# jzi040941/PercepNet

Measured on AMD Instinct MI355X. Metric: real-time 48 kHz streams (10 ms frames), whole job, higher is better.
Workload: dtype f32; 1 GPU; configs[2]: 65536 concurrent 48 kHz streams per MI355X, fp32 network as MFMA GEMM; streams_per_gpu=65536, frame_samples=480, nn_mode=mfma_f32, weights=torch.manual_seed(1234) default-init PercepNet in nnet_data.h layout, parallelism=streams sharded over 1 GPU(s), one process per GPU, no data-path collective, io=int16 PCM in, int16 PCM + g|r rows out, resident in HBM, distributed=none (plain process)

## Files before the change

percepnet_amd/build.py:

```python
import os
import subprocess
import sys

HERE = os.path.dirname(os.path.abspath(__file__))
CSRC = os.path.join(HERE, "csrc")
LIBDIR = os.path.join(HERE, "lib")
LIB = os.path.join(LIBDIR, "libpercepnet_hip.so")
RUN = os.path.join(LIBDIR, "percepnet_run")
EXPORT_MAP = os.path.join(CSRC, "libpercepnet_hip.map")
SOURCES = ["pn_tables.cpp", "pn_model.cpp", "pn_pack.cpp", "pn_dsp_fe.hip", "pn_dsp_fe_g2.hip", "pn_dsp_fe_split_s.hip", "pn_dsp_fe_split_p.hip", "pn_dsp.hip", "pn_outstage.hip", "pn_nn.hip", "pn_nn_small.hip", "pn_nn_x3.hip", "pn_nn_d.hip", "pn_nn_n48.hip", "pn_targets.hip", "pn_state.hip", "pn_active.hip", "pn_stream_state.hip", "pn_context.cpp", "pn_selftest.cpp", "pn_host_pipe.cpp", "pn_stream_state.cpp", "pn_network.cpp",
           "pn_featgen.cpp", "pn_rate.hip", "pn_rate_mix.hip", "pn_rate_plc.hip", "pn_rate_agc.hip", "pn_rate_lim.hip", "pn_rate.cpp", "rnnoise_compat.cpp"]
FLAGS = ["--offload-arch=gfx950", "-O3", "-std=c++17", "-ffp-contract=off", "-fPIC", "-fvisibility=hidden",
         "-Wall", "-Wno-unused-function", "-Wno-unused-variable", "-Wno-unused-value", "-Wno-unused-result"]


EXTRA_FLAGS = {"pn_nn_x3.hip": ["-fno-slp-vectorize", "-mllvm", "-pragma-unroll-threshold=1000000"],
               "pn_nn_d.hip": ["-fno-slp-vectorize"]}


def _hipcc():
    for c in (os.environ.get("HIPCC"), "/opt/rocm/bin/hipcc", "hipcc"):
        if c and (os.path.isabs(c) and os.path.exists(c) or not os.path.isabs(c)):
            return c
    raise RuntimeError("hipcc not found")


EXPECTED_HIP = "7.2"

RESOURCE_LIMITS = {"pn_fe_spec_in_kernel": (0, 0), "pn_fe_spec_out_kernel": (0, 40), "pn_fe_pitch_kernel": (0, 48),
                   "pn_backend_kernel": (0, 16),
                   "pn_gru_x3_kernel": (0, 0), "pn_dense_x3_kernel": (0, 0),
                   "pn_gru_d_kernel": (0, 0),
                   "pn_rate_": (0, 0)}
RESOURCE_SOURCES = ("pn_dsp_fe_split_s.hip", "pn_dsp_fe_split_p.hip", "pn_dsp.hip", "pn_nn_x3.hip", "pn_nn_d.hip", "pn_rate.hip", "pn_rate_mix.hip", "pn_rate_plc.hip", "pn_rate_agc.hip", "pn_rate_lim.hip")


def parse_resource_remarks(text):
    import re
    out, cur = {}, None
    for line in text.splitlines():
        m = re.search(r"remark: .*Function Name: (\S+)", line)
        if m:
            name = m.group(1)
            mm = re.match(r"_Z\d+(pn_[a-z0-9_]+)", name)
            cur = out.setdefault(name, {"kernel": mm.group(1) if mm else name})
            continue
        m = re.search(r"remark: .*?\s+(VGPRs|AGPRs|ScratchSize \[bytes/lane\]|Occupancy \[waves/SIMD\]|LDS Size \[bytes/block\]|VGPRs Spill|SGPRs Spill): (\d+)", line)
        if m and cur is not None:
            cur[m.group(1).split(" [")[0]] = int(m.group(2))
    return out


def check_resources(remarks):
    bad = []
    for name, r in remarks.items():
        for prefix, (max_agpr, max_scratch) in RESOURCE_LIMITS.items():
            if r["kernel"].startswith(prefix):
                if r.get("AGPRs", 0) > max_agpr or r.get("ScratchSize", 0) > max_scratch:
                    bad.append(f"{r['kernel']}: {r.get('VGPRs')} VGPRs, {r.get('AGPRs')} AGPRs, {r.get('ScratchSize')} B/lane scratch "
                               f"(limits: {max_agpr} AGPRs, {max_scratch} B) [{name}]")
    return bad


LLVM_BIN = "/opt/rocm/lib/llvm/bin"
GATED_OBJECTS = ("pn_dsp_fe_split_p",)


def disassemble_device_code(obj_path):
    import shutil
    import tempfile
    objdump = os.path.join(LLVM_BIN, "llvm-objdump")
    if not os.path.exists(objdump):
        objdump = shutil.which("llvm-objdump")
    if not objdump:
        raise RuntimeError("llvm-objdump not found: the disassembly gate cannot run")
    with tempfile.TemporaryDirectory() as d:
        local = os.path.join(d, os.path.basename(obj_path))
        shutil.copy(obj_path, local)
        subprocess.run([objdump, "--offloading", local], cwd=d, capture_output=True, text=True, check=True)
        cos = [f for f in os.listdir(d) if "amdgcn" in f]
        if not cos:
            raise RuntimeError(f"no device code object in {obj_path}")
        return subprocess.run([objdump, "-d", os.path.join(d, cos[0])], capture_output=True, text=True, check=True).stdout


def _vregs(op):
    import re
    m = re.fullmatch(r"v(\d+)", op)
    if m:
        return {int(m.group(1))}
    m = re.fullmatch(r"v\[(\d+):(\d+)\]", op)
    return set(range(int(m.group(1)), int(m.group(2)) + 1)) if m else set()


def check_dpp_and_waitcnt(disasm):
    import re
    bad = []
    func, ins = None, []
    funcs = {}
    for line in disasm.splitlines():
        m = re.match(r"^[0-9a-f]+ <([^>]+)>:", line)
        if m:
            func = m.group(1); ins = funcs.setdefault(func, [])
            continue
        t = line.split("//")[0].strip()
        if func is None or not t or t.startswith("."):
            continue
        parts = t.split(None, 1)
        ops = [o.strip() for o in re.split(r",\s*(?![^\[]*\])", parts[1])] if len(parts) > 1 else []
        ins.append((parts[0], ops, t))
    for func, ins in funcs.items():
        for i, (mn, ops, text) in enumerate(ins):
            if "_dpp" not in mn or len(ops) < 2:
                continue
            src0 = _vregs(ops[1].split()[0])
            if not src0:
                continue
            states, j = 0, i - 1
            while j >= 0 and states < 2:
                pm, pops, ptext = ins[j]
                if pm.startswith("v_") and pops and (_vregs(pops[0].split()[0]) & src0) and not pm.startswith(("v_cmp", "v_nop")):
                    bad.append(f"{func}: `{ptext}` writes the DPP-routed src0 of `{text}` only {states} wait state(s) earlier (need 2)")
                    break
                states += (int(pops[0], 0) + 1) if (pm == "s_nop" and pops) else 1
                j -= 1
        if "pn_fe_pitch_kernel" in func:
            pk = [i for i, x in enumerate(ins) if x[0] == "v_pk_mul_f32"]
            if pk:
                for mn, ops, text in ins[pk[0]:pk[-1] + 1]:
                    if mn.startswith(("s_load_", "s_buffer_load")):
                        bad.append(f"{func}: scalar load `{text}` inside the packed coarse loop (its hand-counted s_waitcnt lgkmcnt(4) assumes LDS reads only)")
    return bad


def toolchain_info(hipcc):
    try:
        out = subprocess.run([hipcc, "--version"], capture_output=True, text=True).stdout
    except OSError as e:
        return f"hipcc --version failed: {e}"
    ver = next((l.split(":", 1)[1].strip() for l in out.splitlines() if l.startswith("HIP version")), "?")
    if not ver.startswith(EXPECTED_HIP):
        print(f"[percepnet_amd.build] WARNING: hipcc reports HIP {ver}; the kernels were validated with HIP {EXPECTED_HIP}.x "
              f"(MFMA-drain and loop back-edge hazards, DESIGN.md): run the GPU parity tests before trusting this build",
              file=sys.stderr, flush=True)
    return out.strip()


def _obj(dirname, src):
    stem, ext = src.rsplit(".", 1)
    return os.path.join(dirname, stem + ("_host" if ext == "cpp" and stem + ".hip" in SOURCES else "") + ".o")


def _stale(target, deps):
    if not os.path.exists(target):
        return True
    t = os.path.getmtime(target)
    return any(os.path.getmtime(d) > t for d in deps)


def build_variant(name, defines, verbose=False, only=None):
    vdir = os.path.join(LIBDIR, "variants", name)
    os.makedirs(vdir, exist_ok=True)
    hipcc = _hipcc()
    objs = []
    for src in SOURCES:
        if only is not None and src not in only:
            objs.append(_obj(LIBDIR, src))
            continue
        o = _obj(vdir, src)
        cmd = [hipcc] + FLAGS + EXTRA_FLAGS.get(src, []) + list(defines) + (["-x", "hip"] if src.endswith(".cpp") else []) + \
              ["-c", os.path.join(CSRC, src), "-o", o]
        if verbose:
            print(" ".join(cmd), flush=True)
        subprocess.check_call(cmd)
        objs.append(o)
    lib = os.path.join(vdir, "libpercepnet_hip.so")
    subprocess.check_call([hipcc, "--offload-arch=gfx950", "-shared", "-fPIC", "-Wl,--version-script=" + EXPORT_MAP, "-o", lib] + objs)
    return lib


def build(force=False, verbose=True):
    os.makedirs(LIBDIR, exist_ok=True)
    hipcc = _hipcc()
    deps = [os.path.join(CSRC, f) for f in os.listdir(CSRC)] + [
        os.path.join(HERE, "..", "include", "percepnet_hip.h"),
        os.path.join(HERE, "..", "include", "percepnet_nnet_data.h")]
    objs = []
    resources = {}
    for src in SOURCES:
        s = os.path.join(CSRC, src)
        o = _obj(LIBDIR, src)
        rlog = o + ".resources.txt"
        if force or _stale(o, deps) or (src in RESOURCE_SOURCES and not os.path.exists(rlog)):
            cmd = [hipcc] + FLAGS + EXTRA_FLAGS.get(src, []) + (["-x", "hip"] if src.endswith(".cpp") else []) + ["-c", s, "-o", o]
            if src in RESOURCE_SOURCES:
                cmd.insert(-4, "-Rpass-analysis=kernel-resource-usage")
            if verbose:
                print(" ".join(cmd), flush=True)
            if src in RESOURCE_SOURCES:
                r = subprocess.run(cmd, capture_output=True, text=True)
                if r.returncode:
                    sys.stderr.write(r.stderr)
                    raise subprocess.CalledProcessError(r.returncode, cmd)
                open(rlog, "w").write("\n".join(l for l in r.stderr.splitlines() if "remark:" in l) + "\n")
            else:
                subprocess.check_call(cmd)
        if src in RESOURCE_SOURCES and os.path.exists(rlog):
            resources.update(parse_resource_remarks(open(rlog).read()))
        objs.append(o)
    bad = check_resources(resources)
    if bad:
        raise RuntimeError("register hygiene gate (build.RESOURCE_LIMITS) failed:\n  " + "\n  ".join(bad))
    for base in GATED_OBJECTS:
        o = os.path.join(LIBDIR, base + ".o")
        stamp = o + ".isa_gate_ok"
        if force or _stale(stamp, [o]):
            viol = check_dpp_and_waitcnt(disassemble_device_code(o))
            if viol:
                raise RuntimeError("disassembly gate (build.check_dpp_and_waitcnt) failed — rebuild with -DPN_FP_DPP_ASM=0 -DPN_FP_COARSE_PK=0 or "
                                   "fix the sequence:\n  " + "\n  ".join(viol[:20]))
            open(stamp, "w").write("ok\n")
    if force or _stale(LIB, objs + [EXPORT_MAP]):
        cmd = [hipcc, "--offload-arch=gfx950", "-shared", "-fPIC", "-Wl,--version-script=" + EXPORT_MAP, "-o", LIB] + objs
        if verbose:
            print(" ".join(cmd), flush=True)
        subprocess.check_call(cmd)
    for name in ("percepnet_run", "percepnet_featgen"):
        cli, exe = os.path.join(CSRC, name + ".cpp"), os.path.join(LIBDIR, name)
        if os.path.exists(cli) and (force or _stale(exe, [cli, LIB])):
            cmd = [hipcc, "--offload-arch=gfx950", "-O2", "-std=c++17", cli, "-o", exe, "-L" + LIBDIR,
                   "-lpercepnet_hip", "-Wl,-rpath,$ORIGIN", "-lpthread"]
            if verbose:
                print(" ".join(cmd), flush=True)
            subprocess.check_call(cmd)
    with open(os.path.join(LIBDIR, "BUILD_INFO.txt"), "w") as f:
        f.write(toolchain_info(hipcc) + "\nflags: " + " ".join(FLAGS) + "\n")
        f.write("DSP kernel resources (hipcc -Rpass-analysis=kernel-resource-usage):\n")
        for name, r in sorted(resources.items(), key=lambda kv: kv[1]["kernel"]):
            f.write(f"  {r['kernel']}: VGPRs {r.get('VGPRs')} AGPRs {r.get('AGPRs')} scratch {r.get('ScratchSize')} B/lane "
                    f"LDS {r.get('LDS Size')} B/block occupancy {r.get('Occupancy')} waves/SIMD  [{name[:60]}]\n")
    return LIB


if __name__ == "__main__":
    build(force="--force" in sys.argv)
    print(LIB)
```

percepnet_amd/csrc/pn_context.cpp:

```cpp
#include "pn_context.h"
#include <stdio.h>
#include <float.h>
#include <math.h>

extern "C" int pn_device_count(void) { int n = 0; return hipGetDeviceCount(&n) == hipSuccess ? n : 0; }


static thread_local bool g_last_alloc_oom = false;
bool &last_alloc_oom() { return g_last_alloc_oom; }
int dev_alloc_into(std::vector<void *> &allocs, size_t &total, hipStream_t stream, void **p, size_t bytes, bool zero) {
  static const bool guard = getenv("PERCEPNET_GUARD") != NULL;
  const size_t pad = guard ? (1u << 20) : 0, body = (bytes + 255) & ~(size_t)255;
  {
    const hipError_t e = hipMalloc(p, guard ? body + pad : bytes);
    if (e != hipSuccess) {
      g_last_alloc_oom = (e == hipErrorOutOfMemory);
      (void)hipGetLastError();
      pn_set_error("hipMalloc(%zu bytes) failed: %s", bytes, hipGetErrorString(e));
      return -1;
    }
  }
  allocs.push_back(*p);
  total += bytes;
  if (zero) PN_HIP_CHECK(hipMemsetAsync(*p, 0, bytes, stream));
  if (guard) PN_HIP_CHECK(hipMemsetAsync((char *)*p + body, 0xFF, pad, stream));
  return 0;
}
#define DEV_ALLOC(ptr, count, zero) \
  do { if (dev_alloc(c, (void **)&(ptr), sizeof(*(ptr)) * (size_t)(count), zero)) goto fail; } while (0)
int tables_upload(std::vector<void *> &allocs, size_t &total, hipStream_t stream, PnTables **tables, float **tansig) {
  PnTables *ht = new PnTables();
  hipError_t e = hipSuccess;
  int rc = pn_build_tables(ht);
  if (!rc) rc = dev_alloc_into(allocs, total, stream, (void **)tables, sizeof(PnTables), false);
  if (!rc) e = hipMemcpyAsync(*tables, ht, sizeof(PnTables), hipMemcpyHostToDevice, stream);
  if (!rc && e == hipSuccess && tansig) {
    rc = dev_alloc_into(allocs, total, stream, (void **)tansig, sizeof(ht->tansig), false);
    if (!rc) e = hipMemcpyAsync(*tansig, ht->tansig, sizeof(ht->tansig), hipMemcpyHostToDevice, stream);
  }
  const hipError_t es = hipStreamSynchronize(stream);
  if (e == hipSuccess) e = es;
  if (!rc && e != hipSuccess) { pn_set_error("table upload failed: %s", hipGetErrorString(e)); rc = -1; }
  delete ht;
  return rc;
}

static int zero_state(pn_ctx *c) {
  for (const pn_ctx::StateBuf &b : c->st) {
    PN_HIP_CHECK(hipMemsetAsync(b.p, 0, b.words * 4, c->stream));
    if (b.sh) PN_HIP_CHECK(hipMemsetAsync(b.sh, 0, b.words * 2 * shadow_halfs_per_element(c), c->stream));
  }
  if (c->lam_mu) PN_HIP_CHECK(hipMemsetAsync(c->lam_mu, 0, (size_t)c->B * sizeof(float2), c->stream));
  c->atten_db.assign(c->B, INFINITY); c->n_limited = 0;
  c->t = 0; c->tn = 0;
  return 0;
}
extern "C" void pn_ctx_destroy(pn_ctx *c) {
  if (!c) return;
  DeviceGuard _dg(c->device);
  hipStreamSynchronize(c->stream);
  pipe_destroy(c);
  for (int k = 1; k < 4; k++) if (c->chain_stream[k]) { hipStreamSynchronize(c->chain_stream[k]); hipStreamDestroy(c->chain_stream[k]); if (c->chain_join[k]) hipEventDestroy(c->chain_join[k]); }
  if (c->chain_fork) hipEventDestroy(c->chain_fork);
  for (auto &e : c->events) { hipEventDestroy(e.a); hipEventDestroy(e.b); }
  for (hipEvent_t e : c->event_pool) hipEventDestroy(e);
  for (void *p : c->allocs) hipFree(p);
  for (pn_ctx::IdRing *r : {&c->ids, &c->act.ids})
    for (auto &sl : r->slot) { if (sl.h) hipHostFree(sl.h); if (sl.ev) hipEventDestroy(sl.ev); }
  weights_release(c);
  if (c->own_stream) hipStreamDestroy(c->stream);
  delete c;
}

extern "C" pn_ctx *pn_ctx_create(const pn_model *model, int device, int n_streams, int nn_mode, void *hip_stream) {
  return ctx_create(model, device, n_streams, nn_mode, hip_stream, true, NULL);
}

int open_device(int device, void *hip_stream, DeviceGuard &guard, hipStream_t *stream, bool *own_stream) {
  int ndev = 0;
  if (hipGetDeviceCount(&ndev) != hipSuccess || ndev <= 0) {
    pn_set_error("no HIP device available (this library has no CPU fallback)");
    return -1;
  }
  if (device < 0 || device >= ndev) { pn_set_error("device %d out of range (%d devices)", device, ndev); return -1; }
  guard.enter(device);
  if (!guard.ok) { pn_set_error("hipSetDevice(%d) failed", device); return -1; }
  *stream = (hipStream_t)hip_stream; *own_stream = !hip_stream;
  if (!hip_stream && hipStreamCreateWithFlags(stream, hipStreamNonBlocking) != hipSuccess) { pn_set_error("hipStreamCreate failed"); return -1; }
  return 0;
}

pn_ctx *ctx_create(const pn_model *model, int device, int n_streams, int nn_mode, void *hip_stream, bool selftest, const PnPlan *plan) {
  if (!model) { pn_set_error("NULL model"); return NULL; }
  if (n_streams < 1) { pn_set_error("n_streams must be >= 1"); return NULL; }
  if (nn_mode != PN_NN_MFMA && nn_mode != PN_NN_STRICT && nn_mode != PN_NN_MFMA_F16 && nn_mode != PN_NN_MFMA_X3) { pn_set_error("bad nn_mode %d", nn_mode); return NULL; }
  DeviceGuard _dg; hipStream_t stream; bool own_stream;
  if (open_device(device, hip_stream, _dg, &stream, &own_stream)) return NULL;
  pn_ctx *c = new pn_ctx();
  c->stream = stream; c->own_stream = own_stream;
  c->device = device; c->B = n_streams; c->Bp = ((size_t)n_streams + 255) / 256 * 256; c->nn_mode = nn_mode; c->plan = plan ? *plan : pn_plan_for(n_streams, nn_mode);
  c->t = 0; c->tn = 0; c->bytes = 0; c->profiling = false;
  memset(c->fam_ms, 0, sizeof(c->fam_ms)); memset(c->fam_n, 0, sizeof(c->fam_n));
  memset(c->L, 0, sizeof(c->L));
  const size_t B = n_streams, Bp = c->Bp;
  float *base[PN_ST_COUNT];
  if (tables_upload(c->allocs, c->bytes, c->stream, &c->tables, &c->tansig)) goto fail;
  for (int e = 0; e < PN_ST_COUNT; e++) {
    pn_ctx::StateBuf &b = c->st[e];
    const PnStateSize z = pn_state_size(pn_kState[e], pn_kState[e].padded ? Bp : B);
    b.words = z.words; b.slot_stride = z.slot_stride;
    DEV_ALLOC(b.p, b.words, false);
    base[e] = b.p;
  }
  c->side = pn_dsp_side(base, nullptr, B);
  for (int e = 0; e < PN_ST_COUNT; e++)
    if (pn_state_shadowed(e, c->plan, nn_mode)) DEV_ALLOC(c->st[e].sh, shadow_halfs_per_element(c) * c->st[e].words, false);
  DEV_ALLOC(c->io_in, B * PN_FRAME, false);
  DEV_ALLOC(c->io_out, B * PN_FRAME, false);
  if (zero_state(c)) goto fail;
  for (int li = 0; li < PN_NLAYERS; li++) { c->geom[li] = model->L[li]; c->geom[li].bias = c->geom[li].w = c->geom[li].rw = NULL; }
  if (weights_acquire(c, model)) goto fail;
  if (hipStreamSynchronize(c->stream) != hipSuccess) { pn_set_error("initial upload failed"); goto fail; }
  if (selftest && (nn_mode == PN_NN_MFMA_X3 || nn_mode == PN_NN_MFMA_F16)) {
    const char *e = getenv("PERCEPNET_X3_SATCOUNT");
    c->x3_sat = e && atoi(e);
  }
  if (selftest && nn_mode != PN_NN_STRICT && nn_selftest(c)) goto fail;
  if (selftest && dsp_selftest(c)) goto fail;
  if (c->x3_sat && pn_x3_sat_set(1)) { pn_set_error("cannot enable the operand-saturation counter"); goto fail; }
  if (c->plan.chains > 1 && chain_streams_init(c)) goto fail;
  return c;
fail:
  pn_ctx_destroy(c);
  return NULL;
}

extern "C" int pn_ctx_reset(pn_ctx *c) { if (!c) return -1; PN_ON_DEVICE(c); if (pipe_drain(c)) return -1; return zero_state(c); }
static int stage_payload_offset(int n) { return (n + 3) & ~3; }
static int id_ring_reserve(pn_ctx *c, pn_ctx::IdRing &r, int cap) {
  if (r.cap >= cap) return 0;
  if (dev_alloc(c, (void **)&r.d, (size_t)cap * sizeof(int), false)) return -1;
  for (auto &sl : r.slot) {
    if (sl.ev) PN_HIP_CHECK(hipEventSynchronize(sl.ev));
    if (sl.h) hipHostFree(sl.h);
    sl.h = NULL;
    PN_HIP_CHECK(hipHostMalloc((void **)&sl.h, (size_t)cap * sizeof(int), hipHostMallocDefault));
    if (!sl.ev) PN_HIP_CHECK(hipEventCreateWithFlags(&sl.ev, hipEventDisableTiming));
  }
  r.cap = cap;
  return 0;
}
static int id_ring_stage(pn_ctx *c, pn_ctx::IdRing &r, const int32_t *ids, int n, const void *payload, int payload_words, int words) {
  auto &sl = r.slot[r.calls++ & 3];
  PN_HIP_CHECK(hipEventSynchronize(sl.ev));
  memcpy(sl.h, ids, (size_t)n * sizeof(int));
  if (payload_words) memcpy(sl.h + stage_payload_offset(n), payload, (size_t)payload_words * 4);
  PN_HIP_CHECK(hipMemcpyAsync(r.d, sl.h, (size_t)words * sizeof(int), hipMemcpyHostToDevice, c->stream));
  PN_HIP_CHECK(hipEventRecord(sl.ev, c->stream));
  return 0;
}
const int *stage_ids(pn_ctx *c, const int32_t *ids, int n, const void *payload, int payload_words) {
  const int words = payload_words ? stage_payload_offset(n) + payload_words : n;
  if (id_ring_reserve(c, c->ids, words < 1024 ? 1024 : words) || id_ring_stage(c, c->ids, ids, n, payload, payload_words, words)) return NULL;
  return c->ids.d;
}
extern "C" int pn_ctx_reset_streams(pn_ctx *c, const int32_t *ids, int n) {
  if (!c) { pn_set_error("bad argument"); return -1; }
  if (pn_ids_check(c->B, ids, n, false)) return -1;
  if (n == 0) return 0;
  PN_ON_DEVICE(c);
  const int *d = stage_ids(c, ids, n);
  if (!d) return -1;
  const int np = (int)shadow_halfs_per_element(c);
  for (int e = 0; e < PN_ST_COUNT; e++) {
    const PnStateEntry &L = pn_kState[e]; const pn_ctx::StateBuf &b = c->st[e];
    const int outer = L.in_row ? 1 : L.slots;
    pn_launch_zero_rows(c->stream, b.p, L.row_words, L.row_words, outer, b.slot_stride, d, n);
    pn_launch_zero_shadow_rows(c->stream, b.sh, L.cols, np, outer, np * b.slot_stride, d, n);
  }
  if (c->lam_mu) pn_launch_zero_rows(c->stream, c->lam_mu, 2, 2, 1, 0, d, n);
  PN_HIP_CHECK(hipGetLastError());
  for (int i = 0; i < n; i++) {
    if (pn_atten_limit_factor(c->atten_db[ids[i]]) != 0.f) c->n_limited--;
    c->atten_db[ids[i]] = INFINITY;
  }
  return 0;
}
extern "C" int pn_ctx_n_streams(const pn_ctx *c) { return c ? c->B : -1; }
extern "C" int64_t pn_ctx_frames_done(const pn_ctx *c) { return c ? c->t : -1; }
extern "C" size_t pn_ctx_device_bytes(const pn_ctx *c) { return c ? c->bytes + ((c->weights && !c->weights_were_cached) ? c->weight_bytes : 0) : 0; }
extern "C" size_t pn_ctx_weight_bytes(const pn_ctx *c) { return (c && c->weights) ? c->weight_bytes : 0; }
extern "C" int pn_ctx_describe(const pn_ctx *c, char *buf, size_t n) {
  if (!c || !buf || !n) return -1;
  const int f = pn_plan_describe(c->plan, c->nn_mode, buf, n);
  if (f < 0 || (size_t)f >= n) return -1;
  const int k = c->plan.chains;
  const int w = f + snprintf(buf + f, n - f, " weights=%s nn_chains=%d%s%s", c->weights_were_cached ? "shared" : "own", k, k > 1 ? ":" : "", k > 1 ? c->chain_kind + 1 : "");
  if (w < 0 || (size_t)w >= n) return -1;
  if (c->x3_sat) {
    DeviceGuard _dg(c->device);
    hipStreamSynchronize(c->stream);
    const int w2 = snprintf(buf + w, n - w, " x3_saturated=%lld", pn_x3_sat_read());
    return (w2 < 0 || (size_t)(w + w2) >= n) ? -1 : w + w2;
  }
  return w;
}
extern "C" int pn_ctx_synchronize(pn_ctx *c) { if (!c) return -1; PN_ON_DEVICE(c); PN_HIP_CHECK(hipStreamSynchronize(c->stream)); return 0; }


static int flush_events(pn_ctx *c) {
  PN_HIP_CHECK(hipStreamSynchronize(c->stream));
  for (int k = 1; k < 4; k++) if (c->chain_stream[k]) PN_HIP_CHECK(hipStreamSynchronize(c->chain_stream[k]));
  for (auto &e : c->events) {
    float ms = 0;
    if (hipEventElapsedTime(&ms, e.a, e.b) == hipSuccess) { c->fam_ms[e.fam] += ms; c->fam_n[e.fam]++; }
    c->event_pool.push_back(e.a); c->event_pool.push_back(e.b);
  }
  c->events.clear();
  return 0;
}

extern "C" int pn_ctx_set_profiling(pn_ctx *c, int enable) {
  if (!c) return -1;
  if (enable && c->event_pool.size() < 2048) {
    PN_ON_DEVICE(c);
    while (c->event_pool.size() < 2048) { hipEvent_t e; PN_HIP_CHECK(hipEventCreate(&e)); c->event_pool.push_back(e); }
  }
  c->profiling = enable != 0;
  return 0;
}
extern "C" int pn_kernel_count(void) { return KF_COUNT; }
extern "C" const char *pn_kernel_name(int i) { return (i >= 0 && i < KF_COUNT) ? pn_kFamilyName[i] : NULL; }
extern "C" int pn_ctx_kernel_time(pn_ctx *c, const char *name, double *total_ms, int64_t *launches) {
  if (!c || !name) return -1;
  if (flush_events(c)) return -1;
  for (int i = 0; i < KF_COUNT; i++)
    if (!strcmp(name, pn_kFamilyName[i])) { if (total_ms) *total_ms = c->fam_ms[i]; if (launches) *launches = c->fam_n[i]; return 0; }
  pn_set_error("unknown kernel family '%s'", name);
  return -1;
}
extern "C" int pn_ctx_reset_profile(pn_ctx *c) {
  if (!c) return -1;
  if (flush_events(c)) return -1;
  memset(c->fam_ms, 0, sizeof(c->fam_ms)); memset(c->fam_n, 0, sizeof(c->fam_n));
  return 0;
}

void pn_launch_fe(hipStream_t st, const PnTables *T, int n_streams, int fe, int k, const PnDspSide &s, const PnDspSlots &sl, const PnDspIn &in, int grid_cap) {
  static PnFeLaunch *const launch[][3] = {{pn_launch_frontend}, {pn_launch_frontend_g2}, {pn_launch_fe_spec_in, pn_launch_fe_pitch, pn_launch_fe_spec_out}};
  static_assert(sizeof(launch) / sizeof(launch[0]) == sizeof(pn_kFe) / sizeof(pn_kFe[0]) && sizeof(launch[0]) / sizeof(launch[0][0]) == sizeof(pn_kFe[0].fam) / sizeof(int),
                "one row of launchers per front-end family of pn_kFe");
  launch[fe][k](st, T, n_streams, s, sl, in, grid_cap);
}

int process_dev(pn_ctx *c, const void *d_in, void *d_out, float *d_gr, int is_i16) {
  if (!c || !d_in || !d_out) { pn_set_error("NULL argument"); return -1; }
  PN_ON_DEVICE(c);
  const PnDspSide &s = c->side;
  const PnDspSlots k = pn_dsp_slots(c->t);
  const PnDspIn in = {d_in, is_i16, PN_FRAME, 1.f / 32768.f};
  float *const gr = c->st[PN_ST_GR].p;
  for (int i = 0; i < pn_kFe[c->plan.fe].n; i++) {
    Scope sc(c, pn_kFe[c->plan.fe].fam[i]);
    pn_launch_fe(c->stream, c->tables, c->B, c->plan.fe, i, s, k, in, c->dsp_grid_cap);
  }
  if (launch_rnn(c)) return -1;
  const bool stage = c->report_on || (c->saturate && is_i16), staged_cast = stage && is_i16;
  { Scope sc(c, KF_BACKEND);
    pn_launch_backend(c->stream, c->tables, c->B, pn_dsp_spec(s, k.slot_r), s.Ps, gr, c->postfilter ? pn_dsp_bands(s, k.slot_r) : nullptr, s.silence,
                      c->st[PN_ST_SYNTH].p, staged_cast ? (void *)c->stage_o : d_out, staged_cast ? 0 : is_i16, c->dsp_grid_cap,
                      c->n_limited > 0 ? c->lam_mu : nullptr); }
  if (stage) {
    Scope sc(c, KF_BACKEND);
    pn_launch_outstage(c->stream, c->B, staged_cast ? c->stage_o : (const float *)d_out, s, (k.frame_t + 6) % PN_HIST_FRAMES, gr,
                       is_i16 ? (int16_t *)d_out : nullptr, c->saturate, c->report_on ? c->report : nullptr);
  }
  if (d_gr) PN_HIP_CHECK(hipMemcpyAsync(d_gr, gr, (size_t)c->B * 68 * 4, hipMemcpyDeviceToDevice, c->stream));
  PN_HIP_CHECK(hipGetLastError());
  c->t++; c->tn++;
  if (c->events.size() >= 4096 && flush_events(c)) return -1;
  return 0;
}

extern "C" int pn_ctx_debug_inject_launch_failure(pn_ctx *c, int enable) {
  if (!c) { pn_set_error("NULL argument"); return -1; }
  c->inject_bad_launch = enable != 0;
  return 0;
}

extern "C" int pn_ctx_set_postfilter(pn_ctx *c, int enable) {
  if (!c) { pn_set_error("NULL argument"); return -1; }
  c->postfilter = enable != 0;
  return 0;
}

static int stage_buffers(pn_ctx *c, bool report) {
  if (!c->stage_o && dev_alloc(c, (void **)&c->stage_o, (size_t)c->B * PN_FRAME * sizeof(float), false)) return -1;
  if (report && !c->report && dev_alloc(c, (void **)&c->report, (size_t)c->B * PN_REPORT_WORDS * 4, true)) return -1;
  return 0;
}
extern "C" int pn_ctx_set_report(pn_ctx *c, int enable) {
  if (!c) { pn_set_error("NULL argument"); return -1; }
  if (enable) { PN_ON_DEVICE(c); if (stage_buffers(c, true)) return -1; }
  else c->next_report = NULL;
  c->report_on = enable != 0;
  return 0;
}
extern "C" int pn_ctx_set_output_saturate(pn_ctx *c, int enable) {
  if (!c) { pn_set_error("NULL argument"); return -1; }
  if (enable) { PN_ON_DEVICE(c); if (stage_buffers(c, false)) return -1; }
  c->saturate = enable != 0;
  return 0;
}
static int report_copy(pn_ctx *c, void *dst, hipMemcpyKind kind) {
  if (!c || !dst) { pn_set_error("NULL argument"); return -1; }
  if (!c->report_on) { pn_set_error("the frame report is off (pn_ctx_set_report)"); return -1; }
  PN_ON_DEVICE(c);
  PN_HIP_CHECK(hipMemcpyAsync(dst, c->report, (size_t)c->B * PN_REPORT_WORDS * 4, kind, c->stream));
  if (kind == hipMemcpyDeviceToHost) PN_HIP_CHECK(hipStreamSynchronize(c->stream));
  return 0;
}
extern "C" int pn_ctx_read_report(pn_ctx *c, void *h_report) { return report_copy(c, h_report, hipMemcpyDeviceToHost); }
extern "C" int pn_ctx_read_report_dev(pn_ctx *c, void *d_report) { return report_copy(c, d_report, hipMemcpyDeviceToDevice); }

extern "C" float pn_atten_limit_factor(float db) {
  if (!(db >= 0.f)) return NAN;
  const float lam = (float)pow(10.0, -(double)db / 20.0);
  return lam < FLT_MIN ? 0.f : lam;
}
extern "C" int pn_ctx_set_atten_limit(pn_ctx *c, const int32_t *ids, int n, const float *db) {
  if (!c || (n > 0 && !db)) { pn_set_error("bad argument"); return -1; }
  if (pn_ids_check(c->B, ids, n, true)) return -1;
  if (n == 0) return 0;
  for (int i = 0; i < n; i++) {
    if (!(db[i] >= 0.f)) { pn_set_error("attenuation limit %g dB for stream %d: must be >= 0 (+inf = off)", (double)db[i], ids[i]); return -1; }
  }
  PN_ON_DEVICE(c);
  if (!c->lam_mu && dev_alloc(c, (void **)&c->lam_mu, (size_t)c->B * sizeof(float2), true)) return -1;
  std::vector<float2> lm(n);
  for (int i = 0; i < n; i++) { const float lam = pn_atten_limit_factor(db[i]); lm[i] = make_float2(lam, 1.0f - lam); }
  const int *d = stage_ids(c, ids, n, lm.data(), 2 * n);
  if (!d) return -1;
  pn_launch_scatter_pairs(c->stream, c->lam_mu, d, reinterpret_cast<const float2 *>(d + stage_payload_offset(n)), n);
  PN_HIP_CHECK(hipGetLastError());
  for (int i = 0; i < n; i++) {
    c->n_limited += (lm[i].x != 0.f) - (pn_atten_limit_factor(c->atten_db[ids[i]]) != 0.f);
    c->atten_db[ids[i]] = db[i];
  }
  return 0;
}
extern "C" int pn_ctx_get_atten_limit(const pn_ctx *c, float *h_db) {
  if (!c || !h_db) { pn_set_error("bad argument"); return -1; }
  memcpy(h_db, c->atten_db.data(), (size_t)c->B * sizeof(float));
  return 0;
}

extern "C" int pn_process_f32(pn_ctx *c, const float *d_in, float *d_out, float *d_gr) { return process_dev(c, d_in, d_out, d_gr, 0); }
extern "C" int pn_process_i16(pn_ctx *c, const int16_t *d_in, int16_t *d_out, float *d_gr) { return process_dev(c, d_in, d_out, d_gr, 1); }
extern "C" int pn_process_i16_multi(pn_ctx *c, const int16_t *d_in, int16_t *d_out, float *d_gr, int n_frames) {
  if (!c) return -1;
  const size_t fs = (size_t)c->B * PN_FRAME;
  for (int f = 0; f < n_frames; f++)
    if (process_dev(c, d_in + f * fs, d_out + f * fs, d_gr ? d_gr + (size_t)f * c->B * 68 : NULL, 1)) return -1;
  return 0;
}

int active_check(pn_ctx *c, const int32_t *ids, int n) {
  if (!c) { pn_set_error("bad argument"); return -1; }
  return pn_ids_check(c->B, ids, n, true, &c->act.mark);
}
int process_active(pn_ctx *c, const void *d_in, void *d_out, float *d_gr, int is_i16, const int32_t *ids, int n) {
  if (!c || !d_in || !d_out) { pn_set_error("NULL argument"); return -1; }
  if (active_check(c, ids, n)) return -1;
  const int B = c->B;
  pn_ctx::Active &A = c->act;
  if (n == B) return process_dev(c, d_in, d_out, d_gr, is_i16);
  A.inactive.clear();
  for (int s = 0; s < B; s++) if (!A.mark[s]) A.inactive.push_back(s);
  const int ni = (int)A.inactive.size();
  PN_ON_DEVICE(c);
  if (A.ids.cap < ni) {
    int cap = 1024; while (cap < ni) cap *= 2; if (cap > B) cap = B;
    if (dev_alloc(c, (void **)&A.save_synth, (size_t)cap * PN_FRAME * 4, false) ||
        dev_alloc(c, (void **)&A.save_out, (size_t)cap * PN_FRAME * 4, false) || dev_alloc(c, (void **)&A.save_gr, (size_t)cap * 68 * 4, false) ||
        dev_alloc(c, (void **)&A.save_period, (size_t)cap * 4, false) || dev_alloc(c, (void **)&A.save_gain, (size_t)cap * 4, false) ||
        id_ring_reserve(c, A.ids, cap)) return -1;
  }
  if (id_ring_stage(c, A.ids, A.inactive.data(), ni, NULL, 0, ni)) return -1;
  PnActiveArgs a; memset(&a, 0, sizeof(a));
  a.ids = A.ids.d; a.synth = c->st[PN_ST_SYNTH].p; a.last_period = c->side.last_period; a.last_gain = c->side.last_gain;
  a.out = d_out; a.out_row_words = is_i16 ? PN_FRAME / 2 : PN_FRAME; a.d_gr = d_gr;
  a.save_synth = A.save_synth; a.save_out = A.save_out; a.save_gr = A.save_gr; a.save_period = A.save_period; a.save_gain = A.save_gain;
  state_sections(c, a.sec);
  pn_launch_inactive_save(c->stream, a, ni);
  if (process_dev(c, d_in, d_out, d_gr, is_i16)) {
    a.restore_only = 1;
    pn_launch_inactive_fixup(c->stream, a, ni);
    return -1;
  }
  pn_launch_inactive_fixup(c->stream, a, ni);
  PN_HIP_CHECK(hipGetLastError());
  return 0;
}
extern "C" int pn_process_f32_active(pn_ctx *c, const float *d_in, float *d_out, float *d_gr, const int32_t *ids, int n) { return process_active(c, d_in, d_out, d_gr, 0, ids, n); }
extern "C" int pn_process_i16_active(pn_ctx *c, const int16_t *d_in, int16_t *d_out, float *d_gr, const int32_t *ids, int n) { return process_active(c, d_in, d_out, d_gr, 1, ids, n); }

static int process_host(pn_ctx *c, const void *h_in, void *h_out, float *h_gr, int is_i16) {
  if (!c || !h_in || !h_out) { pn_set_error("NULL argument"); return -1; }
  PN_ON_DEVICE(c);
  if (pipe_drain(c)) return -1;
  const size_t nbytes = (size_t)c->B * PN_FRAME * (is_i16 ? 2 : 4);
  PN_HIP_CHECK(hipMemcpyAsync(c->io_in, h_in, nbytes, hipMemcpyHostToDevice, c->stream));
  if (process_dev(c, c->io_in, c->io_out, NULL, is_i16)) return -1;
  PN_HIP_CHECK(hipMemcpyAsync(h_out, c->io_out, nbytes, hipMemcpyDeviceToHost, c->stream));
  if (h_gr) PN_HIP_CHECK(hipMemcpyAsync(h_gr, c->st[PN_ST_GR].p, (size_t)c->B * 68 * 4, hipMemcpyDeviceToHost, c->stream));
  PN_HIP_CHECK(hipStreamSynchronize(c->stream));
  return 0;
}
extern "C" int pn_process_host_f32(pn_ctx *c, const float *h_in, float *h_out, float *h_gr) { return process_host(c, h_in, h_out, h_gr, 0); }
extern "C" int pn_process_host_i16(pn_ctx *c, const int16_t *h_in, int16_t *h_out, float *h_gr) { return process_host(c, h_in, h_out, h_gr, 1); }

extern "C" int pn_ctx_read_features(pn_ctx *c, float *h_feat, int32_t *h_silence) {
  if (!c) return -1;
  PN_ON_DEVICE(c);
  if (h_feat)
    PN_HIP_CHECK(hipMemcpy2DAsync(h_feat, PN_NFEAT * 4, c->side.feat, PN_FEAT_STRIDE * 4, PN_NFEAT * 4, c->B, hipMemcpyDeviceToHost, c->stream));
  if (h_silence) PN_HIP_CHECK(hipMemcpyAsync(h_silence, c->side.silence, (size_t)c->B * 4, hipMemcpyDeviceToHost, c->stream));
  PN_HIP_CHECK(hipStreamSynchronize(c->stream));
  return 0;
}

extern "C" int pn_ctx_read_features_dev(pn_ctx *c, float *d_feat, int32_t *d_silence) {
  if (!c) return -1;
  PN_ON_DEVICE(c);
  if (d_feat)
    PN_HIP_CHECK(hipMemcpy2DAsync(d_feat, PN_NFEAT * 4, c->side.feat, PN_FEAT_STRIDE * 4, PN_NFEAT * 4, c->B, hipMemcpyDeviceToDevice, c->stream));
  if (d_silence) PN_HIP_CHECK(hipMemcpyAsync(d_silence, c->side.silence, (size_t)c->B * 4, hipMemcpyDeviceToDevice, c->stream));
  return 0;
}

extern "C" int pn_ctx_compute_rnn_host(pn_ctx *c, const float *h_feat, float *h_gr) {
  if (!c || !h_feat || !h_gr) { pn_set_error("NULL argument"); return -1; }
  PN_ON_DEVICE(c);
  if (pipe_drain(c)) return -1;
  PN_HIP_CHECK(hipMemcpy2DAsync(c->side.feat, PN_FEAT_STRIDE * 4, h_feat, PN_NFEAT * 4, PN_NFEAT * 4, c->B, hipMemcpyHostToDevice, c->stream));
  if (launch_rnn(c)) return -1;
  PN_HIP_CHECK(hipMemcpyAsync(h_gr, c->st[PN_ST_GR].p, (size_t)c->B * 68 * 4, hipMemcpyDeviceToHost, c->stream));
  PN_HIP_CHECK(hipStreamSynchronize(c->stream));
  PN_HIP_CHECK(hipGetLastError());
  c->tn++;
  return 0;
}

extern "C" long long pn_ctx_debug_copy(pn_ctx *c, int which, void *dst, long long max_bytes) {
  if (!c || !dst) return -1;
  static const int entry[14] = {PN_ST_FEAT, PN_ST_C1RING, PN_ST_C2RING, PN_ST_C2OUT, PN_ST_GRU1, PN_ST_GRU2, PN_ST_GRU3, PN_ST_GRU_GB, PN_ST_RB,
                                PN_ST_GR, PN_ST_YRING, PN_ST_PS, PN_ST_HIST, PN_ST_LAST_PERIOD};
  if (which < 0 || which >= 14) { pn_set_error("bad debug buffer id"); return -1; }
  const void *src = c->st[entry[which]].p; const size_t n = c->st[entry[which]].words * 4;
  if ((long long)n > max_bytes) { pn_set_error("debug buffer needs %zu bytes", n); return -1; }
  PN_ON_DEVICE(c);
  if (hipStreamSynchronize(c->stream) != hipSuccess) return -1;
  if (hipMemcpy(dst, src, n, hipMemcpyDeviceToHost) != hipSuccess) { pn_set_error("debug copy failed"); return -1; }
  return (long long)n;
}
```

percepnet_amd/csrc/pn_context.h:

```cpp
#pragma once
#include <array>
#include <functional>
#include <tuple>
#include <vector>
#include "pn_host_rules.h"
#include "pn_launch.h"

struct SharedWeights;
typedef std::tuple<std::array<unsigned char, 32>, size_t, int, int, int> WeightsKey;

struct pn_ctx {
  int device, B, nn_mode;
  PnPlan plan;
  size_t Bp;
  hipStream_t stream; bool own_stream;
  hipStream_t chain_stream[4] = {nullptr, nullptr, nullptr, nullptr};
  hipEvent_t chain_fork = nullptr, chain_join[4] = {nullptr, nullptr, nullptr, nullptr};
  char chain_kind[5] = {'-', '-', '-', '-', 0};
  int64_t t;
  int64_t tn;
  size_t bytes;
  PnLayerHost geom[PN_NLAYERS];
  DevLayer L[PN_NLAYERS];
  SharedWeights *weights = NULL; WeightsKey weights_key; bool weights_were_cached = false; size_t weight_bytes = 0;
  struct IdRing { int *d = NULL; int cap = 0; unsigned calls = 0; struct { int *h = NULL; hipEvent_t ev = nullptr; } slot[4]; };
  IdRing ids;
  struct Active {
    IdRing ids;
    float *save_synth = NULL, *save_gr = NULL, *save_gain = NULL; uint32_t *save_out = NULL; int *save_period = NULL;
    std::vector<uint8_t> mark; std::vector<int32_t> inactive;
  } act;
  PnTables *tables; float *tansig;
  struct StateBuf { float *p; uint16_t *sh; size_t words; long long slot_stride; } st[PN_ST_COUNT] = {};
  PnDspSide side;
  float *io_in, *io_out;
  bool postfilter = false;
  float2 *lam_mu = NULL;
  std::vector<float> atten_db;
  int n_limited = 0;
  bool report_on = false, saturate = false;
  float *stage_o = NULL; uint32_t *report = NULL;
  void *next_report = NULL;
  bool x3_sat = false;
  int dsp_grid_cap = 0;
  bool inject_bad_launch = false;
  std::vector<void *> allocs;
  bool profiling;
  struct Ev { int fam; hipEvent_t a, b; };
  std::vector<Ev> events;
  std::vector<hipEvent_t> event_pool;
  double fam_ms[KF_COUNT]; int64_t fam_n[KF_COUNT];
  struct Pipe {
    bool init = false;
    hipStream_t h2d = nullptr, d2h = nullptr;
    hipEvent_t in_ready[2] = {nullptr, nullptr}, done[2] = {nullptr, nullptr}, delivered[2] = {nullptr, nullptr};
    void *in[2] = {nullptr, nullptr}, *out[2] = {nullptr, nullptr};
    float *gr[2] = {nullptr, nullptr};
    uint32_t *report[2] = {nullptr, nullptr};
    int64_t submitted = 0;
    char kind[3] = {'?', '?', 0};
  } pipe;
};

int open_device(int device, void *hip_stream, DeviceGuard &guard, hipStream_t *stream, bool *own_stream);
pn_ctx *ctx_create(const pn_model *model, int device, int n_streams, int nn_mode, void *hip_stream, bool selftest, const PnPlan *plan);
int dev_alloc_into(std::vector<void *> &allocs, size_t &total, hipStream_t stream, void **p, size_t bytes, bool zero);
static inline int dev_alloc(pn_ctx *c, void **p, size_t bytes, bool zero) { return dev_alloc_into(c->allocs, c->bytes, c->stream, p, bytes, zero); }
bool &last_alloc_oom();
int tables_upload(std::vector<void *> &allocs, size_t &total, hipStream_t stream, PnTables **tables, float **tansig);
const int *stage_ids(pn_ctx *c, const int32_t *ids, int n, const void *payload = NULL, int payload_words = 0);
int process_dev(pn_ctx *c, const void *d_in, void *d_out, float *d_gr, int is_i16);
int active_check(pn_ctx *c, const int32_t *ids, int n);
int process_active(pn_ctx *c, const void *d_in, void *d_out, float *d_gr, int is_i16, const int32_t *ids, int n);
int nn_selftest(pn_ctx *c);
int dsp_selftest(pn_ctx *c);
int pipe_make_stream(pn_ctx *c, hipStream_t *out, char how, int prio, char fallback, const std::vector<hipStream_t> &others, char *kind);
struct PipeStaging { void *in[2], *out[2]; size_t bytes; };
typedef int (*PipeBody)(void *arg, void *d_in, void *d_out, float *d_gr);
int pipe_submit(pn_ctx *c, const PipeStaging &st, const void *h_in, void *h_out, float *h_gr, PipeBody body, void *arg);
int pipe_drain(pn_ctx *c);
void pipe_destroy(pn_ctx *c);
int host_records_sync(pn_ctx *c, bool import, void *h_records, size_t bytes, const std::function<int(void *d_records)> &launch,
                      void *h_extra = NULL, size_t extra_bytes = 0);
int weights_acquire(pn_ctx *c, const pn_model *model);
void weights_release(pn_ctx *c);
int chain_streams_init(pn_ctx *c);
int launch_rnn(pn_ctx *c);
int reshadow(pn_ctx *c, hipStream_t st, int e, const float *p, const int *d_ids = NULL, const int *d_status = NULL, int n = 0);

static inline size_t shadow_halfs_per_element(const pn_ctx *c) { return (c->nn_mode == PN_NN_MFMA_X3 || c->plan.direct) ? 2 : 1; }
static inline uint16_t *shadow_at(const pn_ctx *c, int e, const float *p) { return c->st[e].sh ? c->st[e].sh + shadow_halfs_per_element(c) * (size_t)(p - c->st[e].p) : NULL; }
static inline float *state_at(const pn_ctx *c, int e, int j, size_t r0 = 0) {
  const PnStateEntry &L = pn_kState[e];
  const int slot = j < L.live ? (pn_state_first(L, c->t, c->tn) + j) % L.slots : pn_state_write(L, c->t, c->tn);
  return c->st[e].p + slot * c->st[e].slot_stride + r0 * L.row_words;
}
static inline void state_sections(const pn_ctx *c, PnSsSection sec[PN_SS_NSEC]) {
  for (int e = 0; e < PN_ST_COUNT; e++) {
    const PnStateEntry &L = pn_kState[e]; const pn_ctx::StateBuf &b = c->st[e];
    if (L.rec_off >= 0) sec[pn_state_section(e)] = PnSsSection{b.p, (uint4 *)b.sh, L.row_words, b.slot_stride, L.slots, pn_state_first(L, c->t, c->tn), L.live, L.cols, L.rec_off,
                         b.sh ? (int)shadow_halfs_per_element(c) : 0};
  }
}
static inline std::vector<hipStream_t> busy_streams(const pn_ctx *c) {
  std::vector<hipStream_t> v{c->stream};
  for (int k = 1; k < 4; k++) if (c->chain_stream[k]) v.push_back(c->chain_stream[k]);
  if (c->pipe.h2d) v.push_back(c->pipe.h2d);
  if (c->pipe.d2h) v.push_back(c->pipe.d2h);
  return v;
}

struct Scope {
  pn_ctx *c; int fam; hipEvent_t a, b; bool on; hipStream_t st;
  Scope(pn_ctx *c_, int fam_, hipStream_t st_ = nullptr) : c(c_), fam(fam_), on(c_->profiling), st(st_ ? st_ : c_->stream) {
    if (on) {
      auto take = [&](hipEvent_t &e) { if (c->event_pool.empty()) hipEventCreate(&e); else { e = c->event_pool.back(); c->event_pool.pop_back(); } };
      take(a); take(b); hipEventRecord(a, st);
    }
  }
  ~Scope() {
    if (on) { hipEventRecord(b, st); c->events.push_back({fam, a, b}); }
    static const long sync_mask = getenv("PERCEPNET_SYNC_EACH") ? strtol(getenv("PERCEPNET_SYNC_EACH"), NULL, 0) : 0;
    if (sync_mask & (1L << fam)) hipStreamSynchronize(st);
  }
};
```

percepnet_amd/csrc/pn_launch.h:

```cpp
#pragma once
#include "pn_common.h"
#include "pn_network.h"

typedef void PnFeLaunch(hipStream_t st, const PnTables *T, int n_streams, const PnDspSide &s, const PnDspSlots &k, const PnDspIn &in, int grid_cap);
PnFeLaunch pn_launch_frontend;
PnFeLaunch pn_launch_frontend_g2;
PnFeLaunch pn_launch_fe_spec_in, pn_launch_fe_pitch, pn_launch_fe_spec_out;
void pn_launch_fe(hipStream_t st, const PnTables *T, int n_streams, int fe, int k, const PnDspSide &s, const PnDspSlots &sl, const PnDspIn &in, int grid_cap);
void pn_launch_zero_rows(hipStream_t st, void *base, int row_floats, long long row_stride, int n_slots, long long slot_stride,
                         const int *d_ids, int n);
void pn_launch_zero_shadow_rows(hipStream_t st, void *S, int width, int np, int n_slots, long long slot_stride_halfs,
                                const int *d_ids, int n);
void pn_launch_scatter_pairs(hipStream_t st, float2 *dst, const int *d_ids, const float2 *d_vals, int n);
struct PnSsSection { float *base; uint4 *shadow; long long row_stride, slot_stride; int slots, first, live, cols, rec_off, np; };
struct PnActiveArgs {
  const int *ids;
  float *synth; int *last_period; float *last_gain;
  void *out; int out_row_words; float *d_gr;
  float *save_synth; uint32_t *save_out; float *save_gr; int *save_period; float *save_gain;
  PnSsSection sec[PN_SS_NSEC];
  int restore_only;
};
void pn_launch_inactive_save(hipStream_t st, const PnActiveArgs &a, int n);
int pn_launch_spin(hipStream_t st, long long ticks);
void pn_launch_inactive_fixup(hipStream_t st, const PnActiveArgs &a, int n);
struct PnStreamStateArgs {
  PnSsSection sec[PN_SS_NSEC];
  float *last_gain; int *last_period;
  const int *ids;
  void *rec;
  int *status;
  uint32_t hdr[16];
};
void pn_launch_ss_gather(hipStream_t st, const PnStreamStateArgs &a, int n);
void pn_launch_ss_scatter(hipStream_t st, const PnStreamStateArgs &a, int n);
int pn_launch_split_x3_rows(hipStream_t st, const float *src, int ld, int width, void *S, const int *d_ids, const int *d_status, int n, int np);
int pn_launch_split_d_rows(hipStream_t st, const float *src, int ld, int width, void *S, const int *d_ids, const int *d_status, int n);
void pn_launch_targets(hipStream_t st, const PnTables *T, int n_pairs, const float *ex_clean, const float *ex_noisy,
                       const float *ey_look_noisy, const float *aux_clean, const float *aux_noisy,
                       const int *period_noisy, float *records, long long rec_stride, float *gr);
void pn_launch_saturate_i16(hipStream_t st, int n_pairs, const float *in, int16_t *out, long long out_stride);
void pn_launch_backend(hipStream_t st, const PnTables *T, int n_streams, const float2 *Xs, const float2 *Ps,
                       const float *gr, const float *ex_postfilter , const int *silence, float *synth_mem,
                       void *out, int out_is_i16, int grid_cap,
                       const float2 *lam_mu );
void pn_launch_outstage(hipStream_t st, int n_streams, const float *o, const PnDspSide &s, int hist_slot, const float *gr,
                        int16_t *pcm, int saturate, void *report);
enum { PN_FMT_F32 = 0, PN_FMT_I16 = 1, PN_FMT_G711 = 2 };
static inline size_t pn_fmt_bytes(int fmt) { return fmt == PN_FMT_G711 ? 1 : fmt == PN_FMT_I16 ? 2 : 4; }
int pn_launch_rate_up(hipStream_t st, int factor, int fmt, int n_rows, const int *d_ids, const int *d_laws, const void *in, float *out48, float *tail, const float *taps);
int pn_launch_rate_down(hipStream_t st, int factor, int fmt, int n_rows, const int *d_ids, const int *d_laws, const float *in48, void *out, int saturate, float *tail, const float *taps);
void pn_launch_rate_records(hipStream_t st, int factor, int rate_hz, const int *d_ids, int n, float *tail_up, float *tail_down, int td_stride, void *rec, int scatter);
int pn_launch_rate_up_mixed(hipStream_t st, int fmt, int n_rows, const int *d_ids, const int *d_factors, const int *d_laws, const void *in, float *out48, float *tail, const float *taps);
int pn_launch_rate_down_mixed(hipStream_t st, int fmt, int n_rows, const int *d_ids, const int *d_factors, const int *d_laws, const float *in48, void *out, int saturate, float *tail, const float *taps);
void pn_launch_rate_records_dev(hipStream_t st, const int *d_ids, int n, const int *d_factors, int factor, float *tail_up, float *tail_down, int td_stride,
                                void *rec, int stride_words, int *d_status, int scatter);
void pn_launch_rate_set_factors(hipStream_t st, const int *d_ids, const int *d_vals, int n, int *d_factors);
void pn_launch_rate_mix(hipStream_t st, int n_rows, const int *d_ids, const int *d_conf, const int *d_members, const uint32_t *d_stamp, uint32_t tick,
                        const float *in48, float *out48);
void pn_launch_rate_mix_sel(hipStream_t st, int n_rows, const int *d_ids, const int *d_conf, const int *d_members, const uint32_t *d_stamp, uint32_t tick,
                            const float *in48, float *out48, const float *d_gains, const int *d_caps, float *d_level, float hold, void *d_report);
void pn_launch_rate_conf_stamp(hipStream_t st, const int *d_ids, int n, uint32_t *d_stamp, uint32_t tick);
void pn_launch_rate_conf_rows(hipStream_t st, const int *d_touched, const int *d_rows, int k, int *d_members);
void pn_launch_rate_plc(hipStream_t st, int n_rows, const int *d_ids, const uint32_t *d_lost, uint32_t tick, float *x48, float *hist, float *q,
                        void *meta, void *d_report);
void pn_launch_rate_agc(hipStream_t st, int n_rows, const int *d_ids, const float *d_targets, const uint32_t *d_lost, uint32_t tick, const float *params,
                        float *y48, void *state, void *d_report);
void pn_launch_rate_lim(hipStream_t st, int n_rows, const int *d_ids, const float *d_ceilings, const float *params, float *o48, void *state, void *d_report);
struct DevLayer { float *bias, *w, *rw, *wp, *rwp, *wq; };
struct PnLayerLaunch {
  PnSegs A, S;
  const float *bias;
  const void *w, *rw;
  int N, act; const float *tansig;
  float *out; int ldo;
  void *outS; int nts_out;
  const float *h_old; const void *h_oldS;
  int n_rows, rg, np;
};
typedef int PnLayerLauncher(hipStream_t, const PnLayerLaunch &);
PnLayerLauncher pn_launch_dense_strict, pn_launch_gru_strict, pn_launch_dense, pn_launch_gru;
PnLayerLauncher pn_launch_dense_small, pn_launch_gru_small, pn_launch_dense_n16, pn_launch_dense_n48;
PnLayerLauncher pn_launch_dense_x3, pn_launch_gru_x3, pn_launch_gru_d;
size_t pn_packed_halfs_x3(int k_alloc, int ncols, int ct_round, int np );
int pn_pack_weights_x3(const float *W, int K, int k_alloc, int ncols, int ct_round, int np, void *Wp);
int pn_x3_sat_set(int enable);
long long pn_x3_sat_read();
int pn_launch_split_x3(hipStream_t st, const float *src, int ld, int width, void *S, int n_rows_padded, int np);
int pn_launch_split_d(hipStream_t st, const float *src, int ld, int width, void *S, int n_rows);
```

percepnet_amd/csrc/pn_network.cpp:

```cpp
#include "pn_context.h"
#include <map>
#include <mutex>

struct SharedWeights {
  int refs = 0;
  DevLayer L[PN_NLAYERS];
  std::vector<void *> allocs;
  size_t bytes = 0;
};
static std::mutex g_weights_mu;
static std::mutex g_weights_build_mu[16];
static std::map<WeightsKey, SharedWeights *> g_weights;

static int upload_w(pn_ctx *c, SharedWeights *w, float **dst, const float *src, size_t n) {
  if (dev_alloc_into(w->allocs, w->bytes, c->stream, (void **)dst, n * sizeof(float), false)) return -1;
  PN_HIP_CHECK(hipMemcpyAsync(*dst, src, n * sizeof(float), hipMemcpyHostToDevice, c->stream));
  return 0;
}

static SharedWeights *build_weights(pn_ctx *c, const pn_model *model, int nn_mode, int narrow) {
  SharedWeights *w = new SharedWeights();
  memset(w->L, 0, sizeof(w->L));
  for (int li = 0; li < PN_NLAYERS; li++) {
    const PnLayerHost &H = model->L[li]; DevLayer &D = w->L[li];
    size_t nb, nw, nr; pn_layer_floats(H.kind, H.nin, H.nn, H.ks, &nb, &nw, &nr);
    const int fmt = pn_layer_weight_format(nn_mode, narrow, li), gru = H.kind == PN_KIND_GRU, np = pn_weight_planes(nn_mode);
    const int K = H.nin * H.ks, ncols = H.nn * (gru ? 3 : 1);
    auto put = [&](float **dst, const void *src, size_t n_floats) { return upload_w(c, w, dst, (const float *)src, n_floats) || hipStreamSynchronize(c->stream) != hipSuccess; };
    auto pack = [&](float **dst, const float *W, int k, int k_alloc, int ctr, const char *what) {
      if (fmt != PN_WF_X3) {
        std::vector<float> f(pn_packed_floats(k_alloc, ncols, ctr));
        pn_pack_weights(W, k, k_alloc, ncols, ctr, f.data());
        return put(dst, f.data(), f.size());
      }
      std::vector<uint16_t> h(pn_packed_halfs_x3(k, ncols, ctr, np));
      if (pn_pack_weights_x3(W, k, k, ncols, ctr, np, h.data())) { pn_set_error("layer %d has a %sweight outside the fp16 range: the fp16-operand and split-precision modes cannot represent it", li, what); return true; }
      return put(dst, h.data(), h.size() / 2);
    };
    if (upload_w(c, w, &D.bias, H.bias, nb)) goto fail_w;
    if (fmt == PN_WF_RAW) {
      if (upload_w(c, w, &D.w, H.w, nw) || (nr && upload_w(c, w, &D.rw, H.rw, nr))) goto fail_w;
      continue;
    }
    if (pack(&D.wp, H.w, K, pn_net_k(li), pn_layer_ct_round(nn_mode, narrow, li), "")) goto fail_w;
    if (fmt == PN_WF_F32_N16) {
      std::vector<float> pq(pn_packed_floats_n16(K, ncols));
      pn_pack_weights_n16(H.w, K, ncols, pq.data());
      if (put(&D.wq, pq.data(), pq.size())) goto fail_w;
    }
    if (nr && pack(&D.rwp, H.rw, H.nn, H.nn, 1, "recurrent ")) goto fail_w;
  }
  if (hipStreamSynchronize(c->stream) != hipSuccess) { pn_set_error("weight upload failed"); goto fail_w; }
  return w;
fail_w:
  hipStreamSynchronize(c->stream);
  for (void *p : w->allocs) hipFree(p);
  delete w;
  return NULL;
}

int weights_acquire(pn_ctx *c, const pn_model *model) {
  std::array<unsigned char, 32> dig; memcpy(dig.data(), model->sha256, 32);
  c->weights_key = std::make_tuple(dig, model->n_floats, c->device, c->nn_mode, c->plan.narrow);
  std::lock_guard<std::mutex> build_lk(g_weights_build_mu[c->device & 15]);
  {
    std::lock_guard<std::mutex> lk(g_weights_mu);
    auto it = g_weights.find(c->weights_key);
    if (it != g_weights.end()) { c->weights = it->second; c->weights->refs++; c->weights_were_cached = true; }
  }
  if (!c->weights) {
    SharedWeights *w = build_weights(c, model, c->nn_mode, c->plan.narrow);
    if (!w) return -1;
    w->refs = 1; c->weights = w;
    std::lock_guard<std::mutex> lk(g_weights_mu);
    g_weights[c->weights_key] = w;
  }
  memcpy(c->L, c->weights->L, sizeof(c->L));
  c->weight_bytes = c->weights->bytes;
  return 0;
}
void weights_release(pn_ctx *c) {
  std::lock_guard<std::mutex> lk(g_weights_mu);
  if (!c->weights || --c->weights->refs) return;
  for (void *p : c->weights->allocs) hipFree(p);
  g_weights.erase(c->weights_key);
  delete c->weights;
}

static constexpr struct { PnLayerLauncher *dense, *gru; } kLaunchers[] = {
    {pn_launch_dense_strict, pn_launch_gru_strict}, {pn_launch_dense, pn_launch_gru}, {pn_launch_dense, NULL}, {pn_launch_dense_small, pn_launch_gru_small},
    {pn_launch_dense_n16, NULL}, {pn_launch_dense_n48, NULL}, {pn_launch_dense_x3, pn_launch_gru_x3}, {NULL, pn_launch_gru_d}};
constexpr bool launchers_match_rules() {
  for (int k = 0; k < PN_K_COUNT; k++)
    if ((kLaunchers[k].dense != nullptr) != (pn_kKernelRule[k].dense != nullptr) || (kLaunchers[k].gru != nullptr) != (pn_kKernelRule[k].gru != nullptr)) return false;
  return true;
}
static_assert(sizeof(kLaunchers) / sizeof(kLaunchers[0]) == PN_K_COUNT && launchers_match_rules(), "one launcher per form of every kernel kind (pn_kKernelRule)");

int reshadow(pn_ctx *c, hipStream_t st, int e, const float *p, const int *d_ids, const int *d_status, int n) {
  void *S = shadow_at(c, e, p); const int w = pn_kState[e].cols, np = pn_weight_planes(c->nn_mode);
  if (!S) return 0;
  if (pn_mode_x3(c->nn_mode)) return d_ids ? pn_launch_split_x3_rows(st, p, w, w, S, d_ids, d_status, n, np) : pn_launch_split_x3(st, p, w, w, S, (int)c->Bp, np);
  return d_ids ? pn_launch_split_d_rows(st, p, w, w, S, d_ids, d_status, n) : pn_launch_split_d(st, p, w, w, S, (int)c->Bp);
}

static int launch_rnn_rows(pn_ctx *c, size_t r0, size_t nrows, hipStream_t st) {
  const bool strict = c->nn_mode == PN_NN_STRICT;
  int rc = 0;
  for (int li = 0; li < PN_NLAYERS; li++) {
    const PnNetLayer &R = pn_kNet[li]; const DevLayer &W = c->L[li];
    const int k = pn_layer_kernel(c->plan, c->nn_mode, li), fmt = pn_kernel_weight_format(k); const bool gru = R.state >= 0;
    if (rc && R.fam == KF_GRU512) continue;
    Scope sc(c, R.fam, st);
    PnLayerLaunch L = {};
    PnSegs &A = L.A, &S = L.S; A.n = S.n = R.n_in;
    for (int j = 0; j < R.n_in; j++) {
      const int e = R.in[j].entry;
      A.p[j] = state_at(c, e, R.in[j].j, r0); A.ld[j] = S.ld[j] = pn_kState[e].row_words; A.width[j] = S.width[j] = pn_kState[e].cols;
      S.p[j] = reinterpret_cast<const float *>(shadow_at(c, e, A.p[j]));
    }
    if (li == PN_L_FC && strict) A.width[0] = pn_kGeom[li].nin;
    if (li == PN_L_FC && c->inject_bad_launch && !strict) A.width[0] = 96;
    L.bias = W.bias;
    L.w = fmt == PN_WF_RAW ? W.w : (fmt == PN_WF_F32_N16 ? W.wq : W.wp); L.rw = fmt == PN_WF_RAW ? W.rw : W.rwp;
    L.N = pn_kGeom[li].nn; L.act = c->geom[li].act; L.tansig = c->tansig;
    L.out = state_at(c, R.out.entry, R.out.j, r0) + R.out_col; L.ldo = pn_kState[R.out.entry].row_words;
    L.outS = pn_kernel_writes_shadow(k) ? shadow_at(c, R.out.entry, L.out) : NULL;
    L.nts_out = L.outS ? pn_kState[R.out.entry].cols / 32 : 0;
    if (gru) { L.h_old = state_at(c, R.state, 0, r0); L.h_oldS = shadow_at(c, R.state, L.h_old); }
    L.n_rows = (int)nrows; L.rg = c->plan.rg; L.np = pn_weight_planes(c->nn_mode);
    PnLayerLauncher *launch = gru ? kLaunchers[k].gru : kLaunchers[k].dense;
    rc |= launch ? launch(st, L) : pn_kernel_geometry_ok(k, gru, A.n, A.width, L.N);
    if (!pn_kernel_writes_shadow(k)) rc |= reshadow(c, st, R.out.entry, L.out);
  }
  return rc ? -1 : 0;
}

int chain_streams_init(pn_ctx *c) {
  int lo = 0, hi = 0;
  PN_HIP_CHECK(hipDeviceGetStreamPriorityRange(&lo, &hi));
  for (int k = 1; k < c->plan.chains; k++) {
    if (pipe_make_stream(c, &c->chain_stream[k], 'a', hi, 'h', busy_streams(c), &c->chain_kind[k])) return -1;
    PN_HIP_CHECK(hipEventCreateWithFlags(&c->chain_join[k], hipEventDisableTiming));
  }
  PN_HIP_CHECK(hipEventCreateWithFlags(&c->chain_fork, hipEventDisableTiming));
  return 0;
}
static bool chain_ok(hipError_t e, const char *what, int &rc) {
  if (e == hipSuccess) return true;
  if (!rc) pn_set_error("%s failed: %s", what, hipGetErrorString(e));
  rc = -1;
  return false;
}
int launch_rnn(pn_ctx *c) {
  const int n = c->plan.chains;
  if (n <= 1) return launch_rnn_rows(c, 0, c->B, c->stream);
  const size_t B = c->B, share = pn_plan_share(c->plan, B);
  PN_HIP_CHECK(hipEventRecord(c->chain_fork, c->stream));
  int rc = 0;
  bool started[PN_MAX_CHAINS] = {};
  for (int k = n - 1; k >= 0 && !rc; k--) {
    const size_t r0 = share * k, nr = r0 >= B ? 0 : (B - r0 < share ? B - r0 : share);
    if (!nr) continue;
    hipStream_t st = k ? c->chain_stream[k] : c->stream;
    if (k && !(started[k] = chain_ok(hipStreamWaitEvent(st, c->chain_fork, 0), "hipStreamWaitEvent(chain, fork)", rc))) break;
    if (launch_rnn_rows(c, r0, nr, st)) rc = -1;
  }
  for (int k = 1; k < n; k++)
    if (started[k] && chain_ok(hipEventRecord(c->chain_join[k], c->chain_stream[k]), "hipEventRecord(join)", rc))
      chain_ok(hipStreamWaitEvent(c->stream, c->chain_join[k], 0), "hipStreamWaitEvent(stream, join)", rc);
  return rc;
}
```

percepnet_amd/csrc/pn_network.h:

```cpp
#pragma once
#include "pn_dsp_layout.h"
#include "pn_launch_check.h"

struct PnSegs { const float *p[5]; int ld[5]; int width[5]; int n; };

struct PnRef { int entry, j; };
constexpr PnRef pn_ref_new(int e) { return PnRef{e, pn_kState[e].live}; }
struct PnNetLayer {
  int n_in; PnRef in[5];
  PnRef out; int out_col;
  int state;
  int fam;
};
static constexpr PnNetLayer pn_kNet[PN_NLAYERS] = {
    {1, {{PN_ST_FEAT, 0}}, pn_ref_new(PN_ST_C1RING), 0, -1, KF_FC},
    {5, {{PN_ST_C1RING, 0}, {PN_ST_C1RING, 1}, {PN_ST_C1RING, 2}, {PN_ST_C1RING, 3}, pn_ref_new(PN_ST_C1RING)},
     pn_ref_new(PN_ST_C2RING), 0, -1, KF_CONV1},
    {3, {{PN_ST_C2RING, 0}, {PN_ST_C2RING, 1}, pn_ref_new(PN_ST_C2RING)}, {PN_ST_C2OUT, 0}, 0, -1, KF_CONV2},
    {1, {{PN_ST_C2OUT, 0}}, pn_ref_new(PN_ST_GRU1), 0, PN_ST_GRU1, KF_GRU512},
    {1, {pn_ref_new(PN_ST_GRU1)}, pn_ref_new(PN_ST_GRU2), 0, PN_ST_GRU2, KF_GRU512},
    {1, {pn_ref_new(PN_ST_GRU2)}, pn_ref_new(PN_ST_GRU3), 0, PN_ST_GRU3, KF_GRU512},
    {1, {pn_ref_new(PN_ST_GRU3)}, pn_ref_new(PN_ST_GRU_GB), 0, PN_ST_GRU_GB, KF_GRU512},
    {2, {pn_ref_new(PN_ST_GRU3), {PN_ST_C2OUT, 0}}, pn_ref_new(PN_ST_RB), 0, PN_ST_RB, KF_GRU_RB},
    {5, {{PN_ST_C2OUT, 0}, pn_ref_new(PN_ST_GRU1), pn_ref_new(PN_ST_GRU2), pn_ref_new(PN_ST_GRU3), pn_ref_new(PN_ST_GRU_GB)},
     {PN_ST_GR, 0}, 0, -1, KF_FC_GB},
    {1, {pn_ref_new(PN_ST_RB)}, {PN_ST_GR, 0}, PN_NB, -1, KF_FC_RB},
};
constexpr int pn_net_k(int li) { return pn_kNet[li].n_in * pn_kState[pn_kNet[li].in[0].entry].cols; }
constexpr bool pn_net_ok() {
  for (int li = 0; li < PN_NLAYERS; li++) {
    const PnNetLayer &row = pn_kNet[li]; const PnGeom &geo = pn_kGeom[li]; const PnStateEntry &oent = pn_kState[row.out.entry];
    for (int j = 0; j < row.n_in; j++) {
      const PnRef &in = row.in[j];
      if (pn_kState[in.entry].cols != pn_kState[row.in[0].entry].cols || in.j > pn_kState[in.entry].live) return false;
      if (geo.kind == PN_KIND_CONV1D && (row.n_in != geo.ks || geo.ks != pn_kState[in.entry].slots || in.entry != row.in[0].entry || in.j != j)) return false;
    }
    if (li == PN_L_FC ? (pn_net_k(li) != PN_FEAT_STRIDE || geo.nin != PN_NFEAT) : pn_net_k(li) != geo.nin * geo.ks) return false;
    if (row.out_col + geo.nn > oent.cols || (row.out.entry != PN_ST_GR && oent.cols != geo.nn) || oent.row_words != oent.cols) return false;
    if ((geo.kind == PN_KIND_GRU) != (row.state >= 0) || (row.state >= 0 && (row.out.entry != row.state || row.out.j != pn_kState[row.state].live))) return false;
  }
  return pn_kNet[PN_L_FC_RB].out_col == pn_kGeom[PN_L_FC_GB].nn && pn_kGeom[PN_L_FC_GB].nn + pn_kGeom[PN_L_FC_RB].nn == pn_kState[PN_ST_GR].cols;
}
static_assert(pn_net_ok(), "layer wiring (pn_kNet), topology (pn_kGeom) and state table (pn_kState) agree");

enum { PN_K_STRICT, PN_K_BATCH, PN_K_BATCH_SH, PN_K_SMALL, PN_K_N16, PN_K_N48, PN_K_X3, PN_K_DIRECT, PN_K_COUNT };
constexpr bool pn_mode_x3(int nn_mode) { return nn_mode == PN_NN_MFMA_X3 || nn_mode == PN_NN_MFMA_F16; }
constexpr bool pn_layer_narrow(int li) { return pn_kGeom[li].kind == PN_KIND_DENSE && pn_kGeom[li].nn <= 48; }
constexpr int pn_layer_kernel(const PnPlan &p, int nn_mode, int li) {
  const int fp32 = p.small ? PN_K_SMALL : PN_K_BATCH;
  if (nn_mode == PN_NN_STRICT) return PN_K_STRICT;
  if (pn_mode_x3(nn_mode) && li != PN_L_FC && li != PN_L_FC_RB) return PN_K_X3;
  if (pn_kGeom[li].kind == PN_KIND_GRU) return p.direct ? PN_K_DIRECT : (li == PN_L_GRU_RB ? fp32 : (p.small_gru ? PN_K_SMALL : PN_K_BATCH));
  if (pn_layer_narrow(li) && p.narrow == 1) return PN_K_N16;
  if (li == PN_L_FC_GB && p.narrow == 2) return PN_K_N48;
  return p.direct && li == PN_L_CONV2 ? PN_K_BATCH_SH : fp32;
}
constexpr bool pn_kernel_reads_shadows(int k) { return k == PN_K_X3 || k == PN_K_DIRECT; }
constexpr bool pn_kernel_writes_shadow(int k) { return pn_kernel_reads_shadows(k) || k == PN_K_BATCH_SH; }
constexpr bool pn_state_shadowed(int e, const PnPlan &p, int nn_mode) {
  return pn_kState[e].shadow != PN_SH_NONE && (pn_mode_x3(nn_mode) || (p.direct && pn_kState[e].shadow == PN_SH_MODES_DIRECT));
}

enum { PN_WF_RAW, PN_WF_F32, PN_WF_F32_N16, PN_WF_X3 };
constexpr int pn_kernel_weight_format(int k) {
  return k == PN_K_STRICT ? PN_WF_RAW : (k == PN_K_X3 ? PN_WF_X3 : (k == PN_K_N16 || k == PN_K_N48 ? PN_WF_F32_N16 : PN_WF_F32));
}
constexpr int pn_weight_planes(int nn_mode) { return nn_mode == PN_NN_MFMA_X3 ? 2 : 1;  }
constexpr int pn_layer_weight_format(int nn_mode, int narrow, int li) {
  return pn_kernel_weight_format(pn_layer_kernel(PnPlan{0, 0, 0, narrow, 0, 0, 1}, nn_mode, li));
}

struct PnKernelRule { const char *dense, *gru; };
static constexpr PnKernelRule pn_kKernelRule[PN_K_COUNT] = {
    {"pn_launch_dense_strict", "pn_launch_gru_strict"},
    {"pn_launch_dense", "pn_launch_gru"},
    {"pn_launch_dense", NULL},
    {"pn_launch_dense_small", "pn_launch_gru_small"},
    {"pn_launch_dense_n16", NULL},
    {"pn_launch_dense_n48", NULL},
    {"pn_launch_dense_x3", "pn_launch_gru_x3"},
    {NULL, "pn_launch_gru_d"},
};
constexpr const char *pn_kernel_launcher(int k, bool gru) { return gru ? pn_kKernelRule[k].gru : pn_kKernelRule[k].dense; }
constexpr int pn_kernel_ct_round(int k, bool gru, int N) { return gru ? 1 : ((k == PN_K_X3 ? N >= 128 : N % 128 == 0) ? 4 : 2); }
constexpr int pn_layer_ct_round(int nn_mode, int narrow, int li) {
  return pn_kernel_ct_round(pn_layer_kernel(PnPlan{0, 0, 0, narrow, 0, 0, 1}, nn_mode, li), pn_kGeom[li].kind == PN_KIND_GRU, pn_kGeom[li].nn);
}
static inline int pn_kernel_geometry_ok(int k, bool gru, int n_panels, const int *width, int N) {
  const char *who = k >= 0 && k < PN_K_COUNT ? pn_kernel_launcher(k, gru) : NULL;
  if (!who) { pn_set_error("kernel kind %d has no %s launcher", k, gru ? "GRU" : "dense"); return -1; }
  if (k == PN_K_STRICT || (gru && k == PN_K_BATCH)) return 0;
  if (k == PN_K_N16) return pn_check_n16_geometry(who, n_panels, width, N16_DEPTH);
  if (gru) return k == PN_K_SMALL ? pn_check_gru_small_geometry(who, n_panels, width, N) : pn_check_gru_geometry(who, n_panels, width, N);
  const bool fp32 = k == PN_K_BATCH || k == PN_K_BATCH_SH || k == PN_K_SMALL;
  if (pn_check_dense_geometry(who, n_panels, width, !fp32)) return -1;
  if (k == PN_K_BATCH_SH && pn_kernel_ct_round(k, gru, N) != 4) { pn_set_error("%s: a shadow output needs whole 128-column blocks", who); return -1; }
  if (k == PN_K_N48 && (N < 1 || N > PN_N48_COLS)) { pn_set_error("%s: %d output columns (1..%d)", who, N, PN_N48_COLS); return -1; }
  return 0;
}

static inline const char *pn_kernel_kind_name(int k, int nn_mode, int rg, bool gru) {
  static const char *const x3[2][3] = {{"f16_rows32", "f16_rows64", "f16_rows64_paired"}, {"x3_rows32", "x3_rows64", "x3_rows64_paired"}};
  if (k == PN_K_X3) return x3[nn_mode == PN_NN_MFMA_X3][rg == 3 && gru ? 2 : rg >= 2];
  if (k == PN_K_DIRECT) return rg >= 2 ? "direct_rows64" : "direct_rows32";
  return k == PN_K_SMALL ? "small" : (k == PN_K_N16 ? "n16" : (k == PN_K_N48 ? "n48" : "batch"));
}
static inline int pn_plan_describe(const PnPlan &p, int nn_mode, char *buf, size_t n) {
  const char *nn = nn_mode == PN_NN_STRICT ? "strict" : (nn_mode == PN_NN_MFMA_F16 ? "mfma_f16" : (nn_mode == PN_NN_MFMA_X3 ? "mfma_x3" : "mfma_f32"));
  auto name = [&](int li) { return pn_kernel_kind_name(pn_layer_kernel(p, nn_mode, li), nn_mode, p.rg, pn_kGeom[li].kind == PN_KIND_GRU); };
  const int gb = pn_layer_kernel(p, nn_mode, PN_L_FC_GB), rb = pn_layer_kernel(p, nn_mode, PN_L_FC_RB);
  char narrow[32];
  if (gb == rb) snprintf(narrow, sizeof(narrow), "%s", name(PN_L_FC_GB));
  else snprintf(narrow, sizeof(narrow), "fc_gb:%s+fc_rb:%s", gb == PN_K_X3 ? "x3" : name(PN_L_FC_GB), gb == PN_K_X3 && rb != PN_K_N16 ? "fp32" : name(PN_L_FC_RB));
  return snprintf(buf, n, "nn=%s dense=%s gru=%s gru_rb=%s narrow=%s frontend=%s", nn, name(PN_L_CONV1), name(PN_L_GRU1), name(PN_L_GRU_RB), narrow,
                  pn_kFe[p.fe].name);
}
```

percepnet_amd/csrc/pn_nn_n48.hip:

```cpp
#include "pn_nn_common.h"

typedef float floatx4 __attribute__((ext_vector_type(4)));

#define Q_CT 3
#ifndef PN_N48_RGW
#define PN_N48_RGW 2
#endif

template <int RGW> struct QShared {
  float A[2][4 * RGW * 2 * 4 * 16 * 4];
  fvec4 B[2][2][Q_CT][64];
  float tansig[208];
};

template <int NA>
__device__ __forceinline__ void q_load_A(fvec4 (&ra)[NA], const float *__restrict__ p, int ld, int k0, int m0) {
#pragma unroll
  for (int it = 0; it < NA; it++) {
    const int idx = threadIdx.x + NN_THREADS * it;
    ra[it] = *reinterpret_cast<const fvec4 *>(p + (size_t)(m0 + (idx >> 3)) * ld + k0 + 4 * (idx & 7));
  }
}
template <int NA>
__device__ __forceinline__ void q_store_A(float *As, const fvec4 (&ra)[NA]) {
#pragma unroll
  for (int it = 0; it < NA; it++) {
    const int idx = threadIdx.x + NN_THREADS * it;
    const int row = idx >> 3, c = idx & 7;
    float *dst = As + ((((row >> 4) * 2 + (c >> 2)) * 4) * 16 + (row & 15)) * 4 + (c & 3);
    dst[0] = ra[it].x; dst[64] = ra[it].y; dst[128] = ra[it].z; dst[192] = ra[it].w;
  }
}

template <int RGW>
__global__ __launch_bounds__(NN_THREADS) void pn_dense_n48_kernel(
    PnSegs A, const float *__restrict__ Wq, const float *__restrict__ bias, int N, int KT, int tps, int act,
    const float *__restrict__ tansig, float *__restrict__ out, int ldo, int n_rows) {
  __shared__ QShared<RGW> S;
  constexpr int Q_BM = 64 * RGW, NA = 2 * RGW;
  const int tid = threadIdx.x, wave = __builtin_amdgcn_readfirstlane(tid >> 6), lane = tid & 63;
  const int m0 = blockIdx.x * Q_BM, KG = 2 * KT;
  for (int i = tid; i < 201; i += NN_THREADS) S.tansig[i] = tansig[i];
  floatx4 acc[RGW][Q_CT];
#pragma unroll
  for (int ct = 0; ct < Q_CT; ct++) {
    const int col = 16 * ct + (lane & 15);
    const float bv = col < N ? bias[col] : 0.f;
#pragma unroll
    for (int rg = 0; rg < RGW; rg++)
#pragma unroll
      for (int i = 0; i < 4; i++) acc[rg][ct][i] = bv;
  }
  PN_PANEL_LOCALS(A);
  const int t0 = tid < 192 ? 0 : 1, c0 = tid < 192 ? (tid >> 6) : 0;
  const int t1 = 1, c1 = 1 + ((tid & 127) >> 6);
  fvec4 ra0[NA], ra1[NA], rb0[2], rb1[2];
#define Q_LOADB(rb, gg) do { int g_ = (gg); g_ = g_ < KT ? g_ : KT - 1;                                                           \
    (rb)[0] = *reinterpret_cast<const fvec4 *>(Wq + (((size_t)c0 * KG + 2 * g_ + t0) * 64 + lane) * 4);                          \
    (rb)[1] = *reinterpret_cast<const fvec4 *>(Wq + (((size_t)c1 * KG + 2 * g_ + t1) * 64 + lane) * 4); } while (0)
#define Q_STOREB(buf, rb) do { S.B[buf][t0][c0][lane] = (rb)[0]; S.B[buf][t1][c1][lane] = (rb)[1]; } while (0)
#define Q_LOADA(ra, gg) do { int g_ = (gg); g_ = g_ < KT ? g_ : KT - 1; const int sg_ = g_ / tps;                                 \
    q_load_A<NA>(ra, pn_seg_ptr(PN_PANEL_PASS, sg_), pld, (g_ - sg_ * tps) * 32, m0); } while (0)
#define Q_FRAGS(BUF, t, fa, fb) do {                                                                                              \
    _Pragma("unroll") for (int rg = 0; rg < RGW; rg++)                                                                            \
      (fa)[rg] = *reinterpret_cast<const fvec4 *>(&S.A[BUF][((((RGW * wave + rg) * 2 + (t)) * 4) * 16) * 4 + lane * 4]);           \
    _Pragma("unroll") for (int ct = 0; ct < Q_CT; ct++) (fb)[ct] = S.B[BUF][t][ct][lane]; } while (0)
#define Q_MMA(fa, fb) do {                                                                                                        \
    _Pragma("unroll") for (int e = 0; e < 4; e++)                                                                                 \
      _Pragma("unroll") for (int rg = 0; rg < RGW; rg++)                                                                          \
        _Pragma("unroll") for (int ct = 0; ct < Q_CT; ct++)                                                                       \
          acc[rg][ct] = __builtin_amdgcn_mfma_f32_16x16x4f32((fa)[rg][e], (fb)[ct][e], acc[rg][ct], 0, 0, 0); } while (0)
#define Q_INTERVAL(gg, BUF, RFA, RFB, RSA, RSB) do {                                                                              \
    fvec4 fa0[RGW], fb0[Q_CT], fa1[RGW], fb1[Q_CT];                                                                                   \
    Q_FRAGS(BUF, 0, fa0, fb0);                                                                                                    \
    Q_LOADA(RFA, (gg) + 2); Q_LOADB(RFB, (gg) + 2);                                                                               \
    __builtin_amdgcn_sched_barrier(0);                                                                                            \
    Q_FRAGS(BUF, 1, fa1, fb1);                                                                                                    \
    __builtin_amdgcn_sched_barrier(0);                                                                                            \
    Q_MMA(fa0, fb0);                                                                                                              \
    __builtin_amdgcn_sched_barrier(0);                                                                                            \
    q_store_A<NA>(S.A[(BUF) ^ 1], RSA); Q_STOREB((BUF) ^ 1, RSB);                                                                     \
    __builtin_amdgcn_sched_barrier(0);                                                                                            \
    Q_MMA(fa1, fb1);                                                                                                              \
    __syncthreads();                                                                                                              \
  } while (0)
  Q_LOADA(ra0, 0); Q_LOADB(rb0, 0);
  Q_LOADA(ra1, 1); Q_LOADB(rb1, 1);
  q_store_A<NA>(S.A[0], ra0); Q_STOREB(0, rb0);
  __syncthreads();
#pragma unroll 1
  for (int g = 0; g < KT; g += 2) {
    Q_INTERVAL(g, 0, ra0, rb0, ra1, rb1);
    Q_INTERVAL(g + 1, 1, ra1, rb1, ra0, rb0);
  }
#undef Q_INTERVAL
#undef Q_MMA
#undef Q_FRAGS
#undef Q_LOADA
#undef Q_STOREB
#undef Q_LOADB
#pragma unroll
  for (int ct = 0; ct < Q_CT; ct++) {
    const int col = 16 * ct + (lane & 15);
    if (col >= N) continue;
#pragma unroll
    for (int rg = 0; rg < RGW; rg++)
#pragma unroll
      for (int i = 0; i < 4; i++) {
        const int row = m0 + 16 * RGW * wave + 16 * rg + 4 * (lane >> 4) + i;
        if (row < n_rows) out[(size_t)row * ldo + col] = pn_act(acc[rg][ct][i], act, S.tansig);
      }
  }
}

static_assert(16 * Q_CT == PN_N48_COLS, "the rule of the n48 kind (pn_network.h) and the kernel's block agree");
int pn_launch_dense_n48(hipStream_t st, const PnLayerLaunch &L) {
  if (pn_kernel_geometry_ok(PN_K_N48, false, L.A.n, L.A.width, L.N)) return -1;
  const int tps = L.A.width[0] / 32, KT = tps * L.A.n;
  constexpr int Q_BM = 64 * PN_N48_RGW;
  const int n_mt = (L.n_rows + Q_BM - 1) / Q_BM;
  hipLaunchKernelGGL(pn_dense_n48_kernel<PN_N48_RGW>, dim3(n_mt), dim3(NN_THREADS), 0, st, L.A, (const float *)L.w, L.bias, L.N, KT, tps, L.act,
                     L.tansig, L.out, L.ldo, L.n_rows);
  return 0;
}
```

percepnet_amd/csrc/pn_plan.h:

```cpp
#pragma once
#include <stdlib.h>
#include <string.h>
#include "../../include/percepnet_hip.h"

enum { FE_MONO_G4 = 0, FE_MONO_G2 = 1, FE_SPLIT = 2 };
#define PN_MAX_CHAINS 4

struct PnPlan {
  int fe;
  int small, small_gru;
  int narrow;
  int direct;
  int rg;
  int chains;
};

static inline int pn_plan_env(const char *name, int dflt) { const char *e = getenv(name); return e ? atoi(e) : dflt; }

static inline PnPlan pn_plan_for(int n_streams, int nn_mode) {
  const int n = n_streams;
  const bool f32 = nn_mode == PN_NN_MFMA, x3 = nn_mode == PN_NN_MFMA_X3 || nn_mode == PN_NN_MFMA_F16;
  PnPlan p;
  const char *fe = getenv("PERCEPNET_FE"), *g2 = getenv("PERCEPNET_FE_G2");
  if (fe && !strcmp(fe, "split")) p.fe = FE_SPLIT;
  else if (fe && (!strcmp(fe, "mono") || !strcmp(fe, "g4"))) p.fe = FE_MONO_G4;
  else if (fe && !strcmp(fe, "g2")) p.fe = FE_MONO_G2;
  else if (g2) p.fe = atoi(g2) ? FE_MONO_G2 : FE_MONO_G4;
  else p.fe = FE_SPLIT;
  const int small_rows = pn_plan_env("PERCEPNET_SMALL_ROWS", 4096);
  p.small = n <= small_rows;
  p.small_gru = n <= pn_plan_env("PERCEPNET_SMALL_GRU_ROWS", small_rows < 1536 ? small_rows : 1536);
  const bool n16 = nn_mode != PN_NN_STRICT && n <= pn_plan_env("PERCEPNET_N16_ROWS", 20480);
  const bool n48 = f32 && !p.small && !n16 && pn_plan_env("PERCEPNET_N48", 1) != 0;
  p.narrow = n16 ? 1 : (n48 ? 2 : 0);
  p.direct = f32 && !p.small && !p.small_gru && pn_plan_env("PERCEPNET_NN_DIRECT", n >= 24576) != 0;
  const int rg_env = pn_plan_env(p.direct ? "PERCEPNET_NN_DIRECT_RG" : "PERCEPNET_X3_RG", 0);
  if (p.direct) p.rg = (rg_env == 1 || rg_env == 2) ? rg_env : (n >= 32768 ? 2 : 1);
  else if (x3) p.rg = (rg_env >= 1 && rg_env <= 3) ? rg_env : (n >= 32768 ? 2 : 1);
  else p.rg = 0;
  p.chains = 1;
  if (f32 && !p.small && !p.small_gru) {
    const int mt = (n + 127) / 128;
    const bool exact = (n % 32768 == 0) && (mt <= 512 || mt % 512 == 0) && !(p.direct && n >= 65536);
    int k = pn_plan_env("PN_NN_CHAINS", (n > 16384 && !exact) ? 2 : 1);
    if (k < 1) k = 1;
    if (k > PN_MAX_CHAINS) k = PN_MAX_CHAINS;
    while (k > 1 && n < k * 4096) k--;
    p.chains = k;
  }
  return p;
}

static inline size_t pn_plan_tile(const PnPlan &p) { return p.direct ? 128 * (size_t)p.rg : 128; }
static inline size_t pn_plan_share(const PnPlan &p, size_t n_streams) {
  const size_t k = p.chains, tile = pn_plan_tile(p);
  return k > 1 ? ((n_streams + k - 1) / k + tile - 1) / tile * tile : 0;
}
```

Measured before the change: 72650 streams.

## Fuse the fc_gb and fc_rb output heads into one kernel writing the g|r tap

Adds a heads kernel that computes both narrow output dense layers (gain and r-band heads) in one launch, sharing the n48 MFMA sweep factored into a common header. The kernel also writes its activations straight into the caller's g|r output buffer, so the separate device-to-device copy of the gr rows is skipped when heads mode is active. This removes one launch and one extra pass over the gr rows at the cost of a larger kernel and an extra store path. It is enabled by default for f32 plans that use the n48 path.

```diff
diff --git a/percepnet_amd/build.py b/percepnet_amd/build.py
--- a/percepnet_amd/build.py
+++ b/percepnet_amd/build.py
@@ -8,7 +8,7 @@
 LIB = os.path.join(LIBDIR, "libpercepnet_hip.so")
 RUN = os.path.join(LIBDIR, "percepnet_run")
 EXPORT_MAP = os.path.join(CSRC, "libpercepnet_hip.map")
-SOURCES = ["pn_tables.cpp", "pn_model.cpp", "pn_pack.cpp", "pn_dsp_fe.hip", "pn_dsp_fe_g2.hip", "pn_dsp_fe_split_s.hip", "pn_dsp_fe_split_p.hip", "pn_dsp.hip", "pn_outstage.hip", "pn_nn.hip", "pn_nn_small.hip", "pn_nn_x3.hip", "pn_nn_d.hip", "pn_nn_n48.hip", "pn_targets.hip", "pn_state.hip", "pn_active.hip", "pn_stream_state.hip", "pn_context.cpp", "pn_selftest.cpp", "pn_host_pipe.cpp", "pn_stream_state.cpp", "pn_network.cpp",
+SOURCES = ["pn_tables.cpp", "pn_model.cpp", "pn_pack.cpp", "pn_dsp_fe.hip", "pn_dsp_fe_g2.hip", "pn_dsp_fe_split_s.hip", "pn_dsp_fe_split_p.hip", "pn_dsp.hip", "pn_outstage.hip", "pn_nn.hip", "pn_nn_small.hip", "pn_nn_x3.hip", "pn_nn_d.hip", "pn_nn_n48.hip", "pn_nn_heads.hip", "pn_targets.hip", "pn_state.hip", "pn_active.hip", "pn_stream_state.hip", "pn_context.cpp", "pn_selftest.cpp", "pn_host_pipe.cpp", "pn_stream_state.cpp", "pn_network.cpp",
            "pn_featgen.cpp", "pn_rate.hip", "pn_rate_mix.hip", "pn_rate_plc.hip", "pn_rate_agc.hip", "pn_rate_lim.hip", "pn_rate.cpp", "rnnoise_compat.cpp"]
 FLAGS = ["--offload-arch=gfx950", "-O3", "-std=c++17", "-ffp-contract=off", "-fPIC", "-fvisibility=hidden",
          "-Wall", "-Wno-unused-function", "-Wno-unused-variable", "-Wno-unused-value", "-Wno-unused-result"]
diff --git a/percepnet_amd/csrc/pn_context.cpp b/percepnet_amd/csrc/pn_context.cpp
--- a/percepnet_amd/csrc/pn_context.cpp
+++ b/percepnet_amd/csrc/pn_context.cpp
@@ -264,7 +264,8 @@
     Scope sc(c, pn_kFe[c->plan.fe].fam[i]);
     pn_launch_fe(c->stream, c->tables, c->B, c->plan.fe, i, s, k, in, c->dsp_grid_cap);
   }
-  if (launch_rnn(c)) return -1;
+  const bool heads = c->plan.narrow == 3;
+  if (launch_rnn(c, heads ? d_gr : NULL)) return -1;
   const bool stage = c->report_on || (c->saturate && is_i16), staged_cast = stage && is_i16;
   { Scope sc(c, KF_BACKEND);
     pn_launch_backend(c->stream, c->tables, c->B, pn_dsp_spec(s, k.slot_r), s.Ps, gr, c->postfilter ? pn_dsp_bands(s, k.slot_r) : nullptr, s.silence,
@@ -275,7 +276,7 @@
     pn_launch_outstage(c->stream, c->B, staged_cast ? c->stage_o : (const float *)d_out, s, (k.frame_t + 6) % PN_HIST_FRAMES, gr,
                        is_i16 ? (int16_t *)d_out : nullptr, c->saturate, c->report_on ? c->report : nullptr);
   }
-  if (d_gr) PN_HIP_CHECK(hipMemcpyAsync(d_gr, gr, (size_t)c->B * 68 * 4, hipMemcpyDeviceToDevice, c->stream));
+  if (d_gr && !heads) PN_HIP_CHECK(hipMemcpyAsync(d_gr, gr, (size_t)c->B * 68 * 4, hipMemcpyDeviceToDevice, c->stream));
   PN_HIP_CHECK(hipGetLastError());
   c->t++; c->tn++;
   if (c->events.size() >= 4096 && flush_events(c)) return -1;
diff --git a/percepnet_amd/csrc/pn_context.h b/percepnet_amd/csrc/pn_context.h
--- a/percepnet_amd/csrc/pn_context.h
+++ b/percepnet_amd/csrc/pn_context.h
@@ -85,7 +85,7 @@
 int weights_acquire(pn_ctx *c, const pn_model *model);
 void weights_release(pn_ctx *c);
 int chain_streams_init(pn_ctx *c);
-int launch_rnn(pn_ctx *c);
+int launch_rnn(pn_ctx *c, float *tap = NULL);
 int reshadow(pn_ctx *c, hipStream_t st, int e, const float *p, const int *d_ids = NULL, const int *d_status = NULL, int n = 0);
 
 static inline size_t shadow_halfs_per_element(const pn_ctx *c) { return (c->nn_mode == PN_NN_MFMA_X3 || c->plan.direct) ? 2 : 1; }
diff --git a/percepnet_amd/csrc/pn_launch.h b/percepnet_amd/csrc/pn_launch.h
--- a/percepnet_amd/csrc/pn_launch.h
+++ b/percepnet_amd/csrc/pn_launch.h
@@ -77,11 +77,14 @@
   void *outS; int nts_out;
   const float *h_old; const void *h_oldS;
   int n_rows, rg, np;
+  PnSegs A2; const float *bias2; const void *w2; int N2, act2; float *out2;
+  float *tap; int ld_tap;
 };
 typedef int PnLayerLauncher(hipStream_t, const PnLayerLaunch &);
 PnLayerLauncher pn_launch_dense_strict, pn_launch_gru_strict, pn_launch_dense, pn_launch_gru;
 PnLayerLauncher pn_launch_dense_small, pn_launch_gru_small, pn_launch_dense_n16, pn_launch_dense_n48;
 PnLayerLauncher pn_launch_dense_x3, pn_launch_gru_x3, pn_launch_gru_d;
+PnLayerLauncher pn_launch_heads;
 size_t pn_packed_halfs_x3(int k_alloc, int ncols, int ct_round, int np );
 int pn_pack_weights_x3(const float *W, int K, int k_alloc, int ncols, int ct_round, int np, void *Wp);
 int pn_x3_sat_set(int enable);
diff --git a/percepnet_amd/csrc/pn_network.cpp b/percepnet_amd/csrc/pn_network.cpp
--- a/percepnet_amd/csrc/pn_network.cpp
+++ b/percepnet_amd/csrc/pn_network.cpp
@@ -89,7 +89,7 @@
 
 static constexpr struct { PnLayerLauncher *dense, *gru; } kLaunchers[] = {
     {pn_launch_dense_strict, pn_launch_gru_strict}, {pn_launch_dense, pn_launch_gru}, {pn_launch_dense, NULL}, {pn_launch_dense_small, pn_launch_gru_small},
-    {pn_launch_dense_n16, NULL}, {pn_launch_dense_n48, NULL}, {pn_launch_dense_x3, pn_launch_gru_x3}, {NULL, pn_launch_gru_d}};
+    {pn_launch_dense_n16, NULL}, {pn_launch_dense_n48, NULL}, {pn_launch_dense_x3, pn_launch_gru_x3}, {NULL, pn_launch_gru_d}, {pn_launch_heads, NULL}};
 constexpr bool launchers_match_rules() {
   for (int k = 0; k < PN_K_COUNT; k++)
     if ((kLaunchers[k].dense != nullptr) != (pn_kKernelRule[k].dense != nullptr) || (kLaunchers[k].gru != nullptr) != (pn_kKernelRule[k].gru != nullptr)) return false;
@@ -104,33 +104,51 @@
   return d_ids ? pn_launch_split_d_rows(st, p, w, w, S, d_ids, d_status, n) : pn_launch_split_d(st, p, w, w, S, (int)c->Bp);
 }
 
-static int launch_rnn_rows(pn_ctx *c, size_t r0, size_t nrows, hipStream_t st) {
-  const bool strict = c->nn_mode == PN_NN_STRICT;
+static PnLayerLaunch layer_record(pn_ctx *c, int li, int k, size_t r0, size_t nrows) {
+  const PnNetLayer &R = pn_kNet[li]; const DevLayer &W = c->L[li];
+  const int fmt = pn_kernel_weight_format(k); const bool strict = c->nn_mode == PN_NN_STRICT;
+  PnLayerLaunch L = {};
+  PnSegs &A = L.A, &S = L.S; A.n = S.n = R.n_in;
+  for (int j = 0; j < R.n_in; j++) {
+    const int e = R.in[j].entry;
+    A.p[j] = state_at(c, e, R.in[j].j, r0); A.ld[j] = S.ld[j] = pn_kState[e].row_words; A.width[j] = S.width[j] = pn_kState[e].cols;
+    S.p[j] = reinterpret_cast<const float *>(shadow_at(c, e, A.p[j]));
+  }
+  if (li == PN_L_FC && strict) A.width[0] = pn_kGeom[li].nin;
+  if (li == PN_L_FC && c->inject_bad_launch && !strict) A.width[0] = 96;
+  L.bias = W.bias;
+  L.w = fmt == PN_WF_RAW ? W.w : (fmt == PN_WF_F32_N16 ? W.wq : W.wp); L.rw = fmt == PN_WF_RAW ? W.rw : W.rwp;
+  L.N = pn_kGeom[li].nn; L.act = c->geom[li].act; L.tansig = c->tansig;
+  L.out = state_at(c, R.out.entry, R.out.j, r0) + R.out_col; L.ldo = pn_kState[R.out.entry].row_words;
+  L.outS = pn_kernel_writes_shadow(k) ? shadow_at(c, R.out.entry, L.out) : NULL;
+  L.nts_out = L.outS ? pn_kState[R.out.entry].cols / 32 : 0;
+  if (R.state >= 0) { L.h_old = state_at(c, R.state, 0, r0); L.h_oldS = shadow_at(c, R.state, L.h_old); }
+  L.n_rows = (int)nrows; L.rg = c->plan.rg; L.np = pn_weight_planes(c->nn_mode);
+  return L;
+}
+static int launch_heads(pn_ctx *c, size_t r0, size_t nrows, hipStream_t st, float *tap) {
+  Scope sc(c, pn_kNet[PN_L_FC_GB].fam, st);
+  PnLayerLaunch L = layer_record(c, PN_L_FC_GB, PN_K_HEADS, r0, nrows);
+  const PnLayerLaunch L2 = layer_record(c, PN_L_FC_RB, PN_K_HEADS, r0, nrows);
+  L.A2 = L2.A; L.bias2 = L2.bias; L.w2 = L2.w; L.N2 = L2.N; L.act2 = L2.act; L.out2 = L2.out;
+  L.ld_tap = pn_kState[PN_ST_GR].cols; L.tap = tap ? tap + r0 * L.ld_tap : NULL;
+  return pn_launch_heads(st, L);
+}
+
+static int launch_rnn_rows(pn_ctx *c, size_t r0, size_t nrows, hipStream_t st, float *tap) {
   int rc = 0;
   for (int li = 0; li < PN_NLAYERS; li++) {
-    const PnNetLayer &R = pn_kNet[li]; const DevLayer &W = c->L[li];
-    const int k = pn_layer_kernel(c->plan, c->nn_mode, li), fmt = pn_kernel_weight_format(k); const bool gru = R.state >= 0;
+    const PnNetLayer &R = pn_kNet[li];
+    const int k = pn_layer_kernel(c->plan, c->nn_mode, li); const bool gru = R.state >= 0;
     if (rc && R.fam == KF_GRU512) continue;
+    if (k == PN_K_HEADS) {
+      if (li == PN_L_FC_GB) rc |= launch_heads(c, r0, nrows, st, rc ? NULL : tap);
+      continue;
+    }
     Scope sc(c, R.fam, st);
-    PnLayerLaunch L = {};
-    PnSegs &A = L.A, &S = L.S; A.n = S.n = R.n_in;
-    for (int j = 0; j < R.n_in; j++) {
-      const int e = R.in[j].entry;
-      A.p[j] = state_at(c, e, R.in[j].j, r0); A.ld[j] = S.ld[j] = pn_kState[e].row_words; A.width[j] = S.width[j] = pn_kState[e].cols;
-      S.p[j] = reinterpret_cast<const float *>(shadow_at(c, e, A.p[j]));
-    }
-    if (li == PN_L_FC && strict) A.width[0] = pn_kGeom[li].nin;
-    if (li == PN_L_FC && c->inject_bad_launch && !strict) A.width[0] = 96;
-    L.bias = W.bias;
-    L.w = fmt == PN_WF_RAW ? W.w : (fmt == PN_WF_F32_N16 ? W.wq : W.wp); L.rw = fmt == PN_WF_RAW ? W.rw : W.rwp;
-    L.N = pn_kGeom[li].nn; L.act = c->geom[li].act; L.tansig = c->tansig;
-    L.out = state_at(c, R.out.entry, R.out.j, r0) + R.out_col; L.ldo = pn_kState[R.out.entry].row_words;
-    L.outS = pn_kernel_writes_shadow(k) ? shadow_at(c, R.out.entry, L.out) : NULL;
-    L.nts_out = L.outS ? pn_kState[R.out.entry].cols / 32 : 0;
-    if (gru) { L.h_old = state_at(c, R.state, 0, r0); L.h_oldS = shadow_at(c, R.state, L.h_old); }
-    L.n_rows = (int)nrows; L.rg = c->plan.rg; L.np = pn_weight_planes(c->nn_mode);
+    const PnLayerLaunch L = layer_record(c, li, k, r0, nrows);
     PnLayerLauncher *launch = gru ? kLaunchers[k].gru : kLaunchers[k].dense;
-    rc |= launch ? launch(st, L) : pn_kernel_geometry_ok(k, gru, A.n, A.width, L.N);
+    rc |= launch ? launch(st, L) : pn_kernel_geometry_ok(k, gru, L.A.n, L.A.width, L.N);
     if (!pn_kernel_writes_shadow(k)) rc |= reshadow(c, st, R.out.entry, L.out);
   }
   return rc ? -1 : 0;
@@ -152,9 +170,9 @@
   rc = -1;
   return false;
 }
-int launch_rnn(pn_ctx *c) {
+int launch_rnn(pn_ctx *c, float *tap) {
   const int n = c->plan.chains;
-  if (n <= 1) return launch_rnn_rows(c, 0, c->B, c->stream);
+  if (n <= 1) return launch_rnn_rows(c, 0, c->B, c->stream, tap);
   const size_t B = c->B, share = pn_plan_share(c->plan, B);
   PN_HIP_CHECK(hipEventRecord(c->chain_fork, c->stream));
   int rc = 0;
@@ -164,7 +182,7 @@
     if (!nr) continue;
     hipStream_t st = k ? c->chain_stream[k] : c->stream;
     if (k && !(started[k] = chain_ok(hipStreamWaitEvent(st, c->chain_fork, 0), "hipStreamWaitEvent(chain, fork)", rc))) break;
-    if (launch_rnn_rows(c, r0, nr, st)) rc = -1;
+    if (launch_rnn_rows(c, r0, nr, st, tap)) rc = -1;
   }
   for (int k = 1; k < n; k++)
     if (started[k] && chain_ok(hipEventRecord(c->chain_join[k], c->chain_stream[k]), "hipEventRecord(join)", rc))
diff --git a/percepnet_amd/csrc/pn_network.h b/percepnet_amd/csrc/pn_network.h
--- a/percepnet_amd/csrc/pn_network.h
+++ b/percepnet_amd/csrc/pn_network.h
@@ -43,7 +43,7 @@
 }
 static_assert(pn_net_ok(), "layer wiring (pn_kNet), topology (pn_kGeom) and state table (pn_kState) agree");
 
-enum { PN_K_STRICT, PN_K_BATCH, PN_K_BATCH_SH, PN_K_SMALL, PN_K_N16, PN_K_N48, PN_K_X3, PN_K_DIRECT, PN_K_COUNT };
+enum { PN_K_STRICT, PN_K_BATCH, PN_K_BATCH_SH, PN_K_SMALL, PN_K_N16, PN_K_N48, PN_K_X3, PN_K_DIRECT, PN_K_HEADS, PN_K_COUNT };
 constexpr bool pn_mode_x3(int nn_mode) { return nn_mode == PN_NN_MFMA_X3 || nn_mode == PN_NN_MFMA_F16; }
 constexpr bool pn_layer_narrow(int li) { return pn_kGeom[li].kind == PN_KIND_DENSE && pn_kGeom[li].nn <= 48; }
 constexpr int pn_layer_kernel(const PnPlan &p, int nn_mode, int li) {
@@ -53,6 +53,7 @@
   if (pn_kGeom[li].kind == PN_KIND_GRU) return p.direct ? PN_K_DIRECT : (li == PN_L_GRU_RB ? fp32 : (p.small_gru ? PN_K_SMALL : PN_K_BATCH));
   if (pn_layer_narrow(li) && p.narrow == 1) return PN_K_N16;
   if (li == PN_L_FC_GB && p.narrow == 2) return PN_K_N48;
+  if (pn_layer_narrow(li) && p.narrow == 3) return PN_K_HEADS;
   return p.direct && li == PN_L_CONV2 ? PN_K_BATCH_SH : fp32;
 }
 constexpr bool pn_kernel_reads_shadows(int k) { return k == PN_K_X3 || k == PN_K_DIRECT; }
@@ -63,7 +64,7 @@
 
 enum { PN_WF_RAW, PN_WF_F32, PN_WF_F32_N16, PN_WF_X3 };
 constexpr int pn_kernel_weight_format(int k) {
-  return k == PN_K_STRICT ? PN_WF_RAW : (k == PN_K_X3 ? PN_WF_X3 : (k == PN_K_N16 || k == PN_K_N48 ? PN_WF_F32_N16 : PN_WF_F32));
+  return k == PN_K_STRICT ? PN_WF_RAW : (k == PN_K_X3 ? PN_WF_X3 : (k == PN_K_N16 || k == PN_K_N48 || k == PN_K_HEADS ? PN_WF_F32_N16 : PN_WF_F32));
 }
 constexpr int pn_weight_planes(int nn_mode) { return nn_mode == PN_NN_MFMA_X3 ? 2 : 1;  }
 constexpr int pn_layer_weight_format(int nn_mode, int narrow, int li) {
@@ -80,6 +81,7 @@
     {"pn_launch_dense_n48", NULL},
     {"pn_launch_dense_x3", "pn_launch_gru_x3"},
     {NULL, "pn_launch_gru_d"},
+    {"pn_launch_heads", NULL},
 };
 constexpr const char *pn_kernel_launcher(int k, bool gru) { return gru ? pn_kKernelRule[k].gru : pn_kKernelRule[k].dense; }
 constexpr int pn_kernel_ct_round(int k, bool gru, int N) { return gru ? 1 : ((k == PN_K_X3 ? N >= 128 : N % 128 == 0) ? 4 : 2); }
@@ -95,7 +97,7 @@
   const bool fp32 = k == PN_K_BATCH || k == PN_K_BATCH_SH || k == PN_K_SMALL;
   if (pn_check_dense_geometry(who, n_panels, width, !fp32)) return -1;
   if (k == PN_K_BATCH_SH && pn_kernel_ct_round(k, gru, N) != 4) { pn_set_error("%s: a shadow output needs whole 128-column blocks", who); return -1; }
-  if (k == PN_K_N48 && (N < 1 || N > PN_N48_COLS)) { pn_set_error("%s: %d output columns (1..%d)", who, N, PN_N48_COLS); return -1; }
+  if ((k == PN_K_N48 || k == PN_K_HEADS) && (N < 1 || N > PN_N48_COLS)) { pn_set_error("%s: %d output columns (1..%d)", who, N, PN_N48_COLS); return -1; }
   return 0;
 }
 
@@ -103,14 +105,15 @@
   static const char *const x3[2][3] = {{"f16_rows32", "f16_rows64", "f16_rows64_paired"}, {"x3_rows32", "x3_rows64", "x3_rows64_paired"}};
   if (k == PN_K_X3) return x3[nn_mode == PN_NN_MFMA_X3][rg == 3 && gru ? 2 : rg >= 2];
   if (k == PN_K_DIRECT) return rg >= 2 ? "direct_rows64" : "direct_rows32";
-  return k == PN_K_SMALL ? "small" : (k == PN_K_N16 ? "n16" : (k == PN_K_N48 ? "n48" : "batch"));
+  return k == PN_K_SMALL ? "small" : (k == PN_K_N16 ? "n16" : (k == PN_K_N48 ? "n48" : (k == PN_K_HEADS ? "heads" : "batch")));
 }
 static inline int pn_plan_describe(const PnPlan &p, int nn_mode, char *buf, size_t n) {
   const char *nn = nn_mode == PN_NN_STRICT ? "strict" : (nn_mode == PN_NN_MFMA_F16 ? "mfma_f16" : (nn_mode == PN_NN_MFMA_X3 ? "mfma_x3" : "mfma_f32"));
   auto name = [&](int li) { return pn_kernel_kind_name(pn_layer_kernel(p, nn_mode, li), nn_mode, p.rg, pn_kGeom[li].kind == PN_KIND_GRU); };
   const int gb = pn_layer_kernel(p, nn_mode, PN_L_FC_GB), rb = pn_layer_kernel(p, nn_mode, PN_L_FC_RB);
-  char narrow[32];
-  if (gb == rb) snprintf(narrow, sizeof(narrow), "%s", name(PN_L_FC_GB));
+  char narrow[48];
+  if (gb == PN_K_HEADS) snprintf(narrow, sizeof(narrow), "fc_gb:n48+fc_rb:batch heads=1");
+  else if (gb == rb) snprintf(narrow, sizeof(narrow), "%s", name(PN_L_FC_GB));
   else snprintf(narrow, sizeof(narrow), "fc_gb:%s+fc_rb:%s", gb == PN_K_X3 ? "x3" : name(PN_L_FC_GB), gb == PN_K_X3 && rb != PN_K_N16 ? "fp32" : name(PN_L_FC_RB));
   return snprintf(buf, n, "nn=%s dense=%s gru=%s gru_rb=%s narrow=%s frontend=%s", nn, name(PN_L_CONV1), name(PN_L_GRU1), name(PN_L_GRU_RB), narrow,
                   pn_kFe[p.fe].name);
diff --git a/percepnet_amd/csrc/pn_nn_heads.hip b/percepnet_amd/csrc/pn_nn_heads.hip
--- /dev/null
+++ b/percepnet_amd/csrc/pn_nn_heads.hip
@@ -0,0 +1,68 @@
+#include "pn_nn_n48.h"
+
+template <int RGW>
+__device__ __forceinline__ void h_bias(floatx4 (&acc)[RGW][Q_CT], const float *__restrict__ bias, int N, int lane) {
+#pragma unroll
+  for (int ct = 0; ct < Q_CT; ct++) {
+    const int col = 16 * ct + (lane & 15);
+    const float bv = col < N ? bias[col] : 0.f;
+#pragma unroll
+    for (int rg = 0; rg < RGW; rg++)
+#pragma unroll
+      for (int i = 0; i < 4; i++) acc[rg][ct][i] = bv;
+  }
+}
+template <int RGW>
+__device__ __forceinline__ void h_store(const floatx4 (&acc)[RGW][Q_CT], int N, int act, const float *tab, float *__restrict__ out,
+                                        int ldo, float *__restrict__ tap, int ld_tap, int row0, int n_rows, int lane) {
+#pragma unroll
+  for (int ct = 0; ct < Q_CT; ct++) {
+    const int col = 16 * ct + (lane & 15);
+    if (col >= N) continue;
+#pragma unroll
+    for (int rg = 0; rg < RGW; rg++)
+#pragma unroll
+      for (int i = 0; i < 4; i++) {
+        const int row = row0 + 16 * rg + 4 * (lane >> 4) + i;
+        if (row < n_rows) {
+          const float v = pn_act(acc[rg][ct][i], act, tab);
+          out[(size_t)row * ldo + col] = v;
+          if (tap) tap[(size_t)row * ld_tap + col] = v;
+        }
+      }
+  }
+}
+
+template <int RGW>
+__global__ __launch_bounds__(NN_THREADS) void pn_heads_kernel(
+    PnSegs A, const float *__restrict__ Wq, const float *__restrict__ bias, int N, int KT, int tps, int act,
+    const float *__restrict__ A2, int ld2, const float *__restrict__ Wq2, const float *__restrict__ bias2, int N2, int KT2, int act2, int col2,
+    const float *__restrict__ tansig, float *__restrict__ out, int ldo, float *__restrict__ tap, int ld_tap, int n_rows) {
+  __shared__ QShared<RGW> S;
+  constexpr int Q_BM = 64 * RGW;
+  const int tid = threadIdx.x, wave = __builtin_amdgcn_readfirstlane(tid >> 6), lane = tid & 63;
+  const int m0 = blockIdx.x * Q_BM, row0 = m0 + 16 * RGW * wave;
+  for (int i = tid; i < 201; i += NN_THREADS) S.tansig[i] = tansig[i];
+  floatx4 acc[RGW][Q_CT];
+  h_bias<RGW>(acc, bias, N, lane);
+  {
+    PN_PANEL_LOCALS(A);
+    q_sweep<RGW>(S, acc, PN_PANEL_PASS, Wq, KT, tps, m0, wave, lane);
+  }
+  h_store<RGW>(acc, N, act, S.tansig, out, ldo, tap, ld_tap, row0, n_rows, lane);
+  h_bias<RGW>(acc, bias2, N2, lane);
+  q_sweep<RGW>(S, acc, A2, A2, A2, A2, A2, ld2, Wq2, KT2, KT2, m0, wave, lane);
+  h_store<RGW>(acc, N2, act2, S.tansig, out + col2, ldo, tap ? tap + col2 : nullptr, ld_tap, row0, n_rows, lane);
+}
+
+int pn_launch_heads(hipStream_t st, const PnLayerLaunch &L) {
+  if (pn_kernel_geometry_ok(PN_K_HEADS, false, L.A.n, L.A.width, L.N) || pn_kernel_geometry_ok(PN_K_HEADS, false, L.A2.n, L.A2.width, L.N2)) return -1;
+  if (L.A2.n != 1 || !L.out2 || L.out2 < L.out) { pn_set_error("pn_launch_heads: the second layer reads one panel and writes behind the first"); return -1; }
+  const int tps = L.A.width[0] / 32, KT = tps * L.A.n, KT2 = L.A2.width[0] / 32;
+  constexpr int Q_BM = 64 * PN_N48_RGW;
+  const int n_mt = (L.n_rows + Q_BM - 1) / Q_BM;
+  hipLaunchKernelGGL(pn_heads_kernel<PN_N48_RGW>, dim3(n_mt), dim3(NN_THREADS), 0, st, L.A, (const float *)L.w, L.bias, L.N, KT, tps, L.act,
+                     L.A2.p[0], L.A2.ld[0], (const float *)L.w2, L.bias2, L.N2, KT2, L.act2, (int)(L.out2 - L.out),
+                     L.tansig, L.out, L.ldo, L.tap, L.ld_tap, L.n_rows);
+  return 0;
+}
diff --git a/percepnet_amd/csrc/pn_nn_n48.h b/percepnet_amd/csrc/pn_nn_n48.h
--- /dev/null
+++ b/percepnet_amd/csrc/pn_nn_n48.h
@@ -0,0 +1,89 @@
+#pragma once
+#include "pn_nn_common.h"
+
+typedef float floatx4 __attribute__((ext_vector_type(4)));
+
+#define Q_CT 3
+#ifndef PN_N48_RGW
+#define PN_N48_RGW 2
+#endif
+static_assert(16 * Q_CT == PN_N48_COLS, "the rule of the n48 and heads kinds (pn_network.h) and the kernels' block agree");
+
+template <int RGW> struct QShared {
+  float A[2][4 * RGW * 2 * 4 * 16 * 4];
+  fvec4 B[2][2][Q_CT][64];
+  float tansig[208];
+};
+
+template <int NA>
+__device__ __forceinline__ void q_load_A(fvec4 (&ra)[NA], const float *__restrict__ p, int ld, int k0, int m0) {
+#pragma unroll
+  for (int it = 0; it < NA; it++) {
+    const int idx = threadIdx.x + NN_THREADS * it;
+    ra[it] = *reinterpret_cast<const fvec4 *>(p + (size_t)(m0 + (idx >> 3)) * ld + k0 + 4 * (idx & 7));
+  }
+}
+template <int NA>
+__device__ __forceinline__ void q_store_A(float *As, const fvec4 (&ra)[NA]) {
+#pragma unroll
+  for (int it = 0; it < NA; it++) {
+    const int idx = threadIdx.x + NN_THREADS * it;
+    const int row = idx >> 3, c = idx & 7;
+    float *dst = As + ((((row >> 4) * 2 + (c >> 2)) * 4) * 16 + (row & 15)) * 4 + (c & 3);
+    dst[0] = ra[it].x; dst[64] = ra[it].y; dst[128] = ra[it].z; dst[192] = ra[it].w;
+  }
+}
+
+template <int RGW>
+__device__ __forceinline__ void q_sweep(QShared<RGW> &S, floatx4 (&acc)[RGW][Q_CT], PN_PANEL_ARGS, const float *__restrict__ Wq,
+                                        int KT, int tps, int m0, int wave, int lane) {
+  constexpr int NA = 2 * RGW;
+  const int tid = threadIdx.x, KG = 2 * KT;
+  const int t0 = tid < 192 ? 0 : 1, c0 = tid < 192 ? (tid >> 6) : 0;
+  const int t1 = 1, c1 = 1 + ((tid & 127) >> 6);
+  fvec4 ra0[NA], ra1[NA], rb0[2], rb1[2];
+#define Q_LOADB(rb, gg) do { int g_ = (gg); g_ = g_ < KT ? g_ : KT - 1;                                                           \
+    (rb)[0] = *reinterpret_cast<const fvec4 *>(Wq + (((size_t)c0 * KG + 2 * g_ + t0) * 64 + lane) * 4);                          \
+    (rb)[1] = *reinterpret_cast<const fvec4 *>(Wq + (((size_t)c1 * KG + 2 * g_ + t1) * 64 + lane) * 4); } while (0)
+#define Q_STOREB(buf, rb) do { S.B[buf][t0][c0][lane] = (rb)[0]; S.B[buf][t1][c1][lane] = (rb)[1]; } while (0)
+#define Q_LOADA(ra, gg) do { int g_ = (gg); g_ = g_ < KT ? g_ : KT - 1; const int sg_ = g_ / tps;                                 \
+    q_load_A<NA>(ra, pn_seg_ptr(PN_PANEL_PASS, sg_), pld, (g_ - sg_ * tps) * 32, m0); } while (0)
+#define Q_FRAGS(BUF, t, fa, fb) do {                                                                                              \
+    _Pragma("unroll") for (int rg = 0; rg < RGW; rg++)                                                                            \
+      (fa)[rg] = *reinterpret_cast<const fvec4 *>(&S.A[BUF][((((RGW * wave + rg) * 2 + (t)) * 4) * 16) * 4 + lane * 4]);           \
+    _Pragma("unroll") for (int ct = 0; ct < Q_CT; ct++) (fb)[ct] = S.B[BUF][t][ct][lane]; } while (0)
+#define Q_MMA(fa, fb) do {                                                                                                        \
+    _Pragma("unroll") for (int e = 0; e < 4; e++)                                                                                 \
+      _Pragma("unroll") for (int rg = 0; rg < RGW; rg++)                                                                          \
+        _Pragma("unroll") for (int ct = 0; ct < Q_CT; ct++)                                                                       \
+          acc[rg][ct] = __builtin_amdgcn_mfma_f32_16x16x4f32((fa)[rg][e], (fb)[ct][e], acc[rg][ct], 0, 0, 0); } while (0)
+#define Q_INTERVAL(gg, BUF, RFA, RFB, RSA, RSB) do {                                                                              \
+    fvec4 fa0[RGW], fb0[Q_CT], fa1[RGW], fb1[Q_CT];                                                                                   \
+    Q_FRAGS(BUF, 0, fa0, fb0);                                                                                                    \
+    Q_LOADA(RFA, (gg) + 2); Q_LOADB(RFB, (gg) + 2);                                                                               \
+    __builtin_amdgcn_sched_barrier(0);                                                                                            \
+    Q_FRAGS(BUF, 1, fa1, fb1);                                                                                                    \
+    __builtin_amdgcn_sched_barrier(0);                                                                                            \
+    Q_MMA(fa0, fb0);                                                                                                              \
+    __builtin_amdgcn_sched_barrier(0);                                                                                            \
+    q_store_A<NA>(S.A[(BUF) ^ 1], RSA); Q_STOREB((BUF) ^ 1, RSB);                                                                     \
+    __builtin_amdgcn_sched_barrier(0);                                                                                            \
+    Q_MMA(fa1, fb1);                                                                                                              \
+    __syncthreads();                                                                                                              \
+  } while (0)
+  Q_LOADA(ra0, 0); Q_LOADB(rb0, 0);
+  Q_LOADA(ra1, 1); Q_LOADB(rb1, 1);
+  q_store_A<NA>(S.A[0], ra0); Q_STOREB(0, rb0);
+  __syncthreads();
+#pragma unroll 1
+  for (int g = 0; g < KT; g += 2) {
+    Q_INTERVAL(g, 0, ra0, rb0, ra1, rb1);
+    Q_INTERVAL(g + 1, 1, ra1, rb1, ra0, rb0);
+  }
+#undef Q_INTERVAL
+#undef Q_MMA
+#undef Q_FRAGS
+#undef Q_LOADA
+#undef Q_STOREB
+#undef Q_LOADB
+}
diff --git a/percepnet_amd/csrc/pn_nn_n48.hip b/percepnet_amd/csrc/pn_nn_n48.hip
--- a/percepnet_amd/csrc/pn_nn_n48.hip
+++ b/percepnet_amd/csrc/pn_nn_n48.hip
@@ -1,45 +1,13 @@
-#include "pn_nn_common.h"
-
-typedef float floatx4 __attribute__((ext_vector_type(4)));
-
-#define Q_CT 3
-#ifndef PN_N48_RGW
-#define PN_N48_RGW 2
-#endif
-
-template <int RGW> struct QShared {
-  float A[2][4 * RGW * 2 * 4 * 16 * 4];
-  fvec4 B[2][2][Q_CT][64];
-  float tansig[208];
-};
-
-template <int NA>
-__device__ __forceinline__ void q_load_A(fvec4 (&ra)[NA], const float *__restrict__ p, int ld, int k0, int m0) {
-#pragma unroll
-  for (int it = 0; it < NA; it++) {
-    const int idx = threadIdx.x + NN_THREADS * it;
-    ra[it] = *reinterpret_cast<const fvec4 *>(p + (size_t)(m0 + (idx >> 3)) * ld + k0 + 4 * (idx & 7));
-  }
-}
-template <int NA>
-__device__ __forceinline__ void q_store_A(float *As, const fvec4 (&ra)[NA]) {
-#pragma unroll
-  for (int it = 0; it < NA; it++) {
-    const int idx = threadIdx.x + NN_THREADS * it;
-    const int row = idx >> 3, c = idx & 7;
-    float *dst = As + ((((row >> 4) * 2 + (c >> 2)) * 4) * 16 + (row & 15)) * 4 + (c & 3);
-    dst[0] = ra[it].x; dst[64] = ra[it].y; dst[128] = ra[it].z; dst[192] = ra[it].w;
-  }
-}
+#include "pn_nn_n48.h"
 
 template <int RGW>
 __global__ __launch_bounds__(NN_THREADS) void pn_dense_n48_kernel(
     PnSegs A, const float *__restrict__ Wq, const float *__restrict__ bias, int N, int KT, int tps, int act,
     const float *__restrict__ tansig, float *__restrict__ out, int ldo, int n_rows) {
   __shared__ QShared<RGW> S;
-  constexpr int Q_BM = 64 * RGW, NA = 2 * RGW;
+  constexpr int Q_BM = 64 * RGW;
   const int tid = threadIdx.x, wave = __builtin_amdgcn_readfirstlane(tid >> 6), lane = tid & 63;
-  const int m0 = blockIdx.x * Q_BM, KG = 2 * KT;
+  const int m0 = blockIdx.x * Q_BM;
   for (int i = tid; i < 201; i += NN_THREADS) S.tansig[i] = tansig[i];
   floatx4 acc[RGW][Q_CT];
 #pragma unroll
@@ -52,53 +20,7 @@
       for (int i = 0; i < 4; i++) acc[rg][ct][i] = bv;
   }
   PN_PANEL_LOCALS(A);
-  const int t0 = tid < 192 ? 0 : 1, c0 = tid < 192 ? (tid >> 6) : 0;
-  const int t1 = 1, c1 = 1 + ((tid & 127) >> 6);
-  fvec4 ra0[NA], ra1[NA], rb0[2], rb1[2];
-#define Q_LOADB(rb, gg) do { int g_ = (gg); g_ = g_ < KT ? g_ : KT - 1;                                                           \
-    (rb)[0] = *reinterpret_cast<const fvec4 *>(Wq + (((size_t)c0 * KG + 2 * g_ + t0) * 64 + lane) * 4);                          \
-    (rb)[1] = *reinterpret_cast<const fvec4 *>(Wq + (((size_t)c1 * KG + 2 * g_ + t1) * 64 + lane) * 4); } while (0)
-#define Q_STOREB(buf, rb) do { S.B[buf][t0][c0][lane] = (rb)[0]; S.B[buf][t1][c1][lane] = (rb)[1]; } while (0)
-#define Q_LOADA(ra, gg) do { int g_ = (gg); g_ = g_ < KT ? g_ : KT - 1; const int sg_ = g_ / tps;                                 \
-    q_load_A<NA>(ra, pn_seg_ptr(PN_PANEL_PASS, sg_), pld, (g_ - sg_ * tps) * 32, m0); } while (0)
-#define Q_FRAGS(BUF, t, fa, fb) do {                                                                                              \
-    _Pragma("unroll") for (int rg = 0; rg < RGW; rg++)                                                                            \
-      (fa)[rg] = *reinterpret_cast<const fvec4 *>(&S.A[BUF][((((RGW * wave + rg) * 2 + (t)) * 4) * 16) * 4 + lane * 4]);           \
-    _Pragma("unroll") for (int ct = 0; ct < Q_CT; ct++) (fb)[ct] = S.B[BUF][t][ct][lane]; } while (0)
-#define Q_MMA(fa, fb) do {                                                                                                        \
-    _Pragma("unroll") for (int e = 0; e < 4; e++)                                                                                 \
-      _Pragma("unroll") for (int rg = 0; rg < RGW; rg++)                                                                          \
-        _Pragma("unroll") for (int ct = 0; ct < Q_CT; ct++)                                                                       \
-          acc[rg][ct] = __builtin_amdgcn_mfma_f32_16x16x4f32((fa)[rg][e], (fb)[ct][e], acc[rg][ct], 0, 0, 0); } while (0)
-#define Q_INTERVAL(gg, BUF, RFA, RFB, RSA, RSB) do {                                                                              \
-    fvec4 fa0[RGW], fb0[Q_CT], fa1[RGW], fb1[Q_CT];                                                                                   \
-    Q_FRAGS(BUF, 0, fa0, fb0);                                                                                                    \
-    Q_LOADA(RFA, (gg) + 2); Q_LOADB(RFB, (gg) + 2);                                                                               \
-    __builtin_amdgcn_sched_barrier(0);                                                                                            \
-    Q_FRAGS(BUF, 1, fa1, fb1);                                                                                                    \
-    __builtin_amdgcn_sched_barrier(0);                                                                                            \
-    Q_MMA(fa0, fb0);                                                                                                              \
-    __builtin_amdgcn_sched_barrier(0);                                                                                            \
-    q_store_A<NA>(S.A[(BUF) ^ 1], RSA); Q_STOREB((BUF) ^ 1, RSB);                                                                     \
-    __builtin_amdgcn_sched_barrier(0);                                                                                            \
-    Q_MMA(fa1, fb1);                                                                                                              \
-    __syncthreads();                                                                                                              \
-  } while (0)
-  Q_LOADA(ra0, 0); Q_LOADB(rb0, 0);
-  Q_LOADA(ra1, 1); Q_LOADB(rb1, 1);
-  q_store_A<NA>(S.A[0], ra0); Q_STOREB(0, rb0);
-  __syncthreads();
-#pragma unroll 1
-  for (int g = 0; g < KT; g += 2) {
-    Q_INTERVAL(g, 0, ra0, rb0, ra1, rb1);
-    Q_INTERVAL(g + 1, 1, ra1, rb1, ra0, rb0);
-  }
-#undef Q_INTERVAL
-#undef Q_MMA
-#undef Q_FRAGS
-#undef Q_LOADA
-#undef Q_STOREB
-#undef Q_LOADB
+  q_sweep<RGW>(S, acc, PN_PANEL_PASS, Wq, KT, tps, m0, wave, lane);
 #pragma unroll
   for (int ct = 0; ct < Q_CT; ct++) {
     const int col = 16 * ct + (lane & 15);
@@ -113,7 +35,6 @@
   }
 }
 
-static_assert(16 * Q_CT == PN_N48_COLS, "the rule of the n48 kind (pn_network.h) and the kernel's block agree");
 int pn_launch_dense_n48(hipStream_t st, const PnLayerLaunch &L) {
   if (pn_kernel_geometry_ok(PN_K_N48, false, L.A.n, L.A.width, L.N)) return -1;
   const int tps = L.A.width[0] / 32, KT = tps * L.A.n;
diff --git a/percepnet_amd/csrc/pn_plan.h b/percepnet_amd/csrc/pn_plan.h
--- a/percepnet_amd/csrc/pn_plan.h
+++ b/percepnet_amd/csrc/pn_plan.h
@@ -32,7 +32,8 @@
   p.small_gru = n <= pn_plan_env("PERCEPNET_SMALL_GRU_ROWS", small_rows < 1536 ? small_rows : 1536);
   const bool n16 = nn_mode != PN_NN_STRICT && n <= pn_plan_env("PERCEPNET_N16_ROWS", 20480);
   const bool n48 = f32 && !p.small && !n16 && pn_plan_env("PERCEPNET_N48", 1) != 0;
-  p.narrow = n16 ? 1 : (n48 ? 2 : 0);
+  const bool heads = n48 && pn_plan_env("PERCEPNET_NN_HEADS", 1) != 0;
+  p.narrow = n16 ? 1 : (heads ? 3 : (n48 ? 2 : 0));
   p.direct = f32 && !p.small && !p.small_gru && pn_plan_env("PERCEPNET_NN_DIRECT", n >= 24576) != 0;
   const int rg_env = pn_plan_env(p.direct ? "PERCEPNET_NN_DIRECT_RG" : "PERCEPNET_X3_RG", 0);
   if (p.direct) p.rg = (rg_env == 1 || rg_env == 2) ? rg_env : (n >= 32768 ? 2 : 1);
```

Result: no change. 72580 streams, median of 3 (-0.1%).
